# CliMA/ClimaSeaIce.jl

Hardware: AMD Instinct MI355X
Metric: EVP sub-cycle cell-updates/s (higher is better)
Workload: dtype f64; 1 GPU; evp_subcycle_fplane_periodic_2048x2048_as_1x1_tiles_of_2048x2048_120substeps; substeps=120, mode=fast, halo=4, halo_exchange=none (one tile)

## Files before the change

climaseaice.jl_amd/csrc/evp_fast_math.h:

```cpp
#pragma once
#include "csi_dev.h"

namespace csi {
namespace fm {

#define CSI_EPS64 2.220446049250313e-16

__device__ __forceinline__ double fma_(double a, double b, double c) { return __builtin_fma(a, b, c); }
__device__ __forceinline__ double fmax_(double a, double b) { return __builtin_fmax(a, b); }
__device__ __forceinline__ double fmin_(double a, double b) { return __builtin_fmin(a, b); }
__device__ __forceinline__ double clampd(double x, double lo, double hi) { return x > hi ? hi : (x < lo ? lo : x); }
__device__ __forceinline__ double avg2(double a, double b) { return 0.5 * (a + b); }
__device__ __forceinline__ double avg4(double a, double b, double c, double d) { return 0.25 * ((a + b) + (c + d)); }
__device__ __forceinline__ double sum2(double a, double b) { return a + b; }
__device__ __forceinline__ double quarter(double s_a, double s_b) { return 0.25 * (s_a + s_b); }

__device__ __forceinline__ double rcp(double x) {
    const double r = __builtin_amdgcn_rcp(x);
    return fma_(fma_(-x, r, 1.0), r, r);
}
__device__ __forceinline__ double rsqrt(double x) {
    const double y = __builtin_amdgcn_rsq(x);
    const double g = x * y, h = 0.5 * y;
    const double r = fma_(-h, g, 0.5);
    return fma_(y, r, y);
}
__device__ __forceinline__ void sqrt_rsqrt(double x, double& s, double& rs) {
    const double y = __builtin_amdgcn_rsq(x);
    double g = x * y, h = 0.5 * y;
    const double r = fma_(-h, g, 0.5);
    g = fma_(g, r, g);
    h = fma_(h, r, h);
    const double d = fma_(-g, g, x);
    s = fma_(d, h, g);
    rs = 2.0 * h;
}
__device__ __forceinline__ double sqrt_fast(double x) {
    const double y = __builtin_amdgcn_rsq(x);
    const double g = x * y, h = 0.5 * y;
    const double r = fma_(-h, g, 0.5);
    return fma_(g, r, g);
}

template <bool UNI>
__device__ __forceinline__ void strain_cell(double A, double Bn, double Bs, double Cn, double Cs,
                                            double u_e, double u_w, double v_n, double v_s, double& e11, double& e22) {
    if (UNI) {
        e11 = A * (u_e - u_w);
        e22 = Cn * (v_n - v_s);
    } else {
        e11 = fma_(A, u_e - u_w, fma_(Bn, v_n, -(Bs * v_s)));
        e22 = fma_(Cn, v_n, -(Cs * v_s));
    }
}
template <bool UNI>
__device__ __forceinline__ double strain_corner(double Sn, double Ss, double Sv, double u_n, double u_s, double v_e, double v_w) {
    if (UNI) return fma_(Sv, v_e - v_w, Sn * (u_n - u_s));
    return fma_(Sv, v_e - v_w, fma_(Sn, u_n, -(Ss * u_s)));
}

struct StressConst {
    double em2, Dmin, Dmin2, rDmin, amin, amax, amin2, amax2, ramin, ramax;
    double hk1;
    int pressure_kind;
    double em2_8, Dmin2_16;
};

struct StressOut {
    double s11, s22, s12, alpha, zc2, zf2;
    double xc, rDc;
};

__device__ __forceinline__ StressOut stress_update_r(const StressConst& k, double e11c, double e22c, double e12f,
                                                     double e11f, double e22f, double e12c, double Pc, double Pf,
                                                     double mc, double mf, double rmc, double rmf, double hkc, double hkf,
                                                     double s11, double s22, double s12) {
    StressOut o;
    const double dc = e11c + e22c, df = e11f + e22f;
    const double tc = e11c - e22c, tf = e11f - e22f;
    const double sc2 = fma_(tc, tc, 4.0 * (e12c * e12c));
    const double sf2 = fma_(tf, tf, 4.0 * (e12f * e12f));
    const double xc = fmax_(fma_(dc, dc, sc2 * k.em2), k.Dmin2), xf = fmax_(fma_(df, df, sf2 * k.em2), k.Dmin2);
    const double rDc = rsqrt(xc), rDf = rsqrt(xf);
    const double zc2 = Pc * rDc, zf2 = Pf * rDf;
    const double Pr = (k.pressure_kind == 0) ? Pc * rcp(fma_(k.Dmin, rDc, 1.0)) : Pc;
    const double ec2 = zc2 * k.em2, ef2 = zf2 * k.em2;
    const double bulk = fma_(zc2 * k.hk1, dc, -0.5 * Pr);
    const double s11n = fma_(ec2, e11c, bulk);
    const double s22n = fma_(ec2, e22c, bulk);
    const double s12n = ef2 * e12f;
    const double g2c_raw = zc2 * hkc * rmc, g2f_raw = zf2 * hkf * rmf;
    const double g2c = fmax_(fmin_(g2c_raw, k.amax2), k.amin2);
    const double g2f = fmax_(fmin_(g2f_raw, k.amax2), k.amin2);
    double gc, rgc, gf, rgf;
    sqrt_rsqrt(g2c, gc, rgc);
    sqrt_rsqrt(g2f, gf, rgf);
    const double wc = (mc > 0) ? rgc : 0.0, wf = (mf > 0) ? rgf : 0.0;
    o.s11 = fma_(s11n - s11, wc, s11);
    o.s22 = fma_(s22n - s22, wc, s22);
    o.s12 = fma_(s12n - s12, wf, s12);
    o.alpha = gc;
    o.zc2 = zc2; o.zf2 = zf2; o.xc = xc; o.rDc = rDc;
    return o;
}

__device__ __forceinline__ StressOut stress_update_s(const StressConst& k, double e11c, double e22c, double E12f,
                                                     double S11f, double S22f, double y2, double Pc, double XP,
                                                     double mc, double M4, double rmc, double rM4, double hkc, double hkf4,
                                                     double s11, double s22, double s12) {
    StressOut o;
    const double dc = e11c + e22c, DF = S11f + S22f;
    const double tc = e11c - e22c, TF = S11f - S22f;
    const double sc2 = fma_(tc, tc, y2 * y2);
    const double sf2 = fma_(TF, TF, E12f * E12f);
    const double xc = fmax_(fma_(dc, dc, sc2 * k.em2), k.Dmin2), xf = fmax_(fma_(DF, DF, sf2 * k.em2), k.Dmin2_16);
    const double rDc = rsqrt(xc), rDf = rsqrt(xf);
    const double zc2 = Pc * rDc, zf2 = XP * rDf;
    const double Pr = (k.pressure_kind == 0) ? Pc * rcp(fma_(k.Dmin, rDc, 1.0)) : Pc;
    const double ec2 = zc2 * k.em2, ef2 = zf2 * k.em2_8;
    const double bulk = fma_(zc2 * k.hk1, dc, -0.5 * Pr);
    const double s11n = fma_(ec2, e11c, bulk);
    const double s22n = fma_(ec2, e22c, bulk);
    const double s12n = ef2 * E12f;
    const double g2c_raw = zc2 * hkc * rmc, g2f_raw = zf2 * hkf4 * rM4;
    const double g2c = fmax_(fmin_(g2c_raw, k.amax2), k.amin2);
    const double g2f = fmax_(fmin_(g2f_raw, k.amax2), k.amin2);
    double gc, rgc, gf, rgf;
    sqrt_rsqrt(g2c, gc, rgc);
    sqrt_rsqrt(g2f, gf, rgf);
    const double wc = (mc > 0) ? rgc : 0.0, wf = (M4 > 0) ? rgf : 0.0;
    o.s11 = fma_(s11n - s11, wc, s11);
    o.s22 = fma_(s22n - s22, wc, s22);
    o.s12 = fma_(s12n - s12, wf, s12);
    o.alpha = gc;
    o.zc2 = zc2; o.zf2 = zf2; o.xc = xc; o.rDc = rDc;
    return o;
}

__device__ __forceinline__ StressOut stress_update(const StressConst& k, double e11c, double e22c, double e12f,
                                                   double e11f, double e22f, double e12c, double Pc, double Pf,
                                                   double mc, double mf, double hkc, double hkf,
                                                   double s11, double s22, double s12) {
    return stress_update_r(k, e11c, e22c, e12f, e11f, e22f, e12c, Pc, Pf, mc, mf, rcp(mc), rcp(mf), hkc, hkf, s11, s22, s12);
}

struct VelConst {
    double dt, rdt, fcor, min_mass, min_conc;
    int has_cor;
};

__device__ __forceinline__ void ext_stress(int kind, double tau, double rhoCd, double we, double webar, double w, double wbar,
                                           double& ex, double& im) {
    if (kind == 3) {
        const double d1 = we - w, d2 = webar - wbar;
        const double n2 = fma_(d1, d1, d2 * d2);
        const double n = sqrt_fast(fmax_(n2, 2.2250738585072014e-308));
        im = rhoCd * n;
        ex = im * we;
    } else {
        ex = tau; im = 0.0;
    }
}

__device__ __forceinline__ void ext_stress_rest(double rhoCd, double w, double wbar, double& ex, double& im) {
    const double n2 = fma_(w, w, wbar * wbar);
    im = rhoCd * sqrt_fast(fmax_(n2, 2.2250738585072014e-308));
    ex = 0.0;
}

__device__ __forceinline__ double vel_update_avg(const VelConst& k, double w, double wn, double mi, double ai, double abar,
                                                 double div, double cor, double ext, double imt, double exb, double imb, bool peripheral) {
    const double rm = rcp(mi);
    const double rai = rm * ai;
    const double G = fma_(wn - w, k.rdt, fma_(div, rm, fma_(exb - ext, rai, cor)));
    const double tau_i = (imb - imt) * rai;
    const double wD = fma_(k.dt, G, abar * w) * rcp(fma_(k.dt, tau_i, abar));
    const bool active_ice = (mi >= k.min_mass) & (ai >= k.min_conc);
    double res = active_ice ? wD : 0.0;
    return peripheral ? 0.0 : res;
}
__device__ __forceinline__ double vel_update_avg_fd(const VelConst& k, double w, double wn, double mi, double ai, double abar,
                                                    double div, double cor, double ext, double imt, double exb, double imb,
                                                    bool peripheral, double wf) {
    const double wD = vel_update_avg(k, w, wn, mi, ai, abar, div, cor, ext, imt, exb, imb, false);
    const bool active_ice = (mi >= k.min_mass) & (ai >= k.min_conc);
    const bool marginal = (mi > CSI_EPS64) & (ai > CSI_EPS64);
    const double res = active_ice ? wD : (marginal ? wf : 0.0);
    return peripheral ? 0.0 : res;
}
__device__ __forceinline__ double vel_update(const VelConst& k, double w, double wn, double m_a, double m_b, double a_a, double a_b,
                                             double al_a, double al_b, double div, double cor,
                                             double ext, double imt, double exb, double imb, bool peripheral) {
    return vel_update_avg(k, w, wn, avg2(m_a, m_b), avg2(a_a, a_b), avg2(al_a, al_b), div, cor, ext, imt, exb, imb, peripheral);
}
__device__ __forceinline__ double vel_update_fd(const VelConst& k, double w, double wn, double m_a, double m_b, double a_a, double a_b,
                                                double al_a, double al_b, double div, double cor,
                                                double ext, double imt, double exb, double imb, bool peripheral, double wf) {
    return vel_update_avg_fd(k, w, wn, avg2(m_a, m_b), avg2(a_a, a_b), avg2(al_a, al_b), div, cor, ext, imt, exb, imb, peripheral, wf);
}

__device__ __forceinline__ double vel_update_sum(const VelConst& k2, double w, double wn, double m2, double a2, double al2,
                                                 double div2, double cor, double ext, double imt, double exb, double imb, bool peripheral) {
    const double rm2 = rcp(m2);
    const double rai = rm2 * a2;
    const double G = fma_(wn - w, k2.rdt, fma_(div2, rm2, fma_(exb - ext, rai, cor)));
    const double tau_i = (imb - imt) * rai;
    const double wD = fma_(k2.dt, G, al2 * w) * rcp(fma_(k2.dt, tau_i, al2));
    const bool active_ice = (m2 >= k2.min_mass) & (a2 >= k2.min_conc);
    double res = active_ice ? wD : 0.0;
    return peripheral ? 0.0 : res;
}
__device__ __forceinline__ double vel_update_sum_fd(const VelConst& k2, double w, double wn, double m2, double a2, double al2,
                                                    double div2, double cor, double ext, double imt, double exb, double imb,
                                                    bool peripheral, double wf) {
    const double wD = vel_update_sum(k2, w, wn, m2, a2, al2, div2, cor, ext, imt, exb, imb, false);
    const bool active_ice = (m2 >= k2.min_mass) & (a2 >= k2.min_conc);
    const bool marginal = (m2 > 2.0 * CSI_EPS64) & (a2 > 2.0 * CSI_EPS64);
    const double res = active_ice ? wD : (marginal ? wf : 0.0);
    return peripheral ? 0.0 : res;
}

__device__ __forceinline__ double div1(double E, double Fn, double Fs, double s11_0, double s11_m, double s12_p, double s12_0) {
    return fma_(E, s11_0 - s11_m, fma_(Fn, s12_p, -(Fs * s12_0)));
}
template <bool UNI>
__device__ __forceinline__ double div2(double Q1n, double Q2n, double Q1s, double Q2s, double K,
                                       double s11_0, double s22_0, double s11_m, double s22_m, double s12_p, double s12_0) {
    if (UNI) return fma_(K, s12_p - s12_0, Q2n * (s22_0 - s22_m));
    const double n = fma_(Q1n, s11_0, Q2n * s22_0);
    const double s = fma_(Q1s, s11_m, Q2s * s22_m);
    return fma_(K, s12_p - s12_0, n - s);
}

__device__ __forceinline__ void full_strain_cell(double Uy_e, double Uy_w, double Vx_n, double Vx_s, double Ur_e, double Ur_w,
                                                 double Vr_n, double Vr_s, double dyc2, double dxc2, double razc, double& e11, double& e22) {
    const double D1 = (Uy_e - Uy_w) + (Vx_n - Vx_s);
    const double D2 = fma_(dyc2, Ur_e - Ur_w, -(dxc2 * (Vr_n - Vr_s)));
    const double hr = 0.5 * razc;
    e11 = hr * (D1 + D2);
    e22 = hr * (D1 - D2);
}
__device__ __forceinline__ double full_strain_corner(double Ux_n, double Ux_s, double Vy_e, double Vy_w, double dxf2, double dyf2, double razf) {
    return (0.5 * razf) * fma_(dxf2, Ux_n - Ux_s, dyf2 * (Vy_e - Vy_w));
}
__device__ __forceinline__ double full_div1(double dyu, double rdyu, double rdxu, double razu, double S_e, double S_w, double T_e, double T_w,
                                            double Z_n, double Z_s) {
    return razu * fma_(0.5 * dyu, S_e - S_w, fma_(0.5 * rdyu, T_e - T_w, rdxu * (Z_n - Z_s)));
}
__device__ __forceinline__ double full_div2(double dxv, double rdxv, double rdyv, double razv, double S_n, double S_s, double T_n, double T_s,
                                            double Z_e, double Z_w) {
    return razv * fma_(0.5 * dxv, S_n - S_s, fma_(-0.5 * rdxv, T_n - T_s, rdyv * (Z_e - Z_w)));
}

__device__ __forceinline__ double full_strain_corner8(double Ux_n, double Ux_s, double Vy_e, double Vy_w, double dxf2, double dyf2, double razf) {
    return (4.0 * razf) * fma_(dxf2, Ux_n - Ux_s, dyf2 * (Vy_e - Vy_w));
}
__device__ __forceinline__ double full_div1_x2(double dyu, double rdyu, double rdxu, double razu, double S_e, double S_w, double T_e, double T_w,
                                               double Z_n, double Z_s) {
    return razu * fma_(dyu, S_e - S_w, fma_(rdyu, T_e - T_w, (rdxu + rdxu) * (Z_n - Z_s)));
}
__device__ __forceinline__ double full_div2_x2(double dxv, double rdxv, double rdyv, double razv, double S_n, double S_s, double T_n, double T_s,
                                               double Z_e, double Z_w) {
    return razv * fma_(dxv, S_n - S_s, fma_(-rdxv, T_n - T_s, (rdyv + rdyv) * (Z_e - Z_w)));
}

}
}
```

climaseaice.jl_amd/csrc/evp_fused2.hip:

```cpp
#include "evp_pair_stage.h"

#include <cstdio>
#include <cstdlib>

#ifndef CSI_PAIR_WAVES
#define CSI_PAIR_WAVES 3
#endif
#ifndef CSI_PAIR_UNI_WAVES
#define CSI_PAIR_UNI_WAVES 2
#endif
#ifndef CSI_PAIR_FULL_WAVES
#define CSI_PAIR_FULL_WAVES 2
#endif
#ifndef CSI_PAIR_PRIO
#define CSI_PAIR_PRIO 2
#endif
#ifndef CSI_PAIR_HOIST
#define CSI_PAIR_HOIST 1
#endif
#ifndef CSI_FULL_FENCE
#define CSI_FULL_FENCE 1
#endif
#ifndef CSI_PAIR_STORES
#define CSI_PAIR_STORES 7
#endif
#ifndef CSI_PEER_EXP
#define CSI_PEER_EXP 3
#endif
#ifndef CSI_PAIR_SKIPB
#define CSI_PAIR_SKIPB 0
#endif
#ifndef CSI_PAIR_PD
#define CSI_PAIR_PD 1
#endif

namespace csi {
namespace fused {

#ifdef CSI_PAIR_PROBE
static __device__ unsigned long long g_probe[8192 * 16];
#define PROBE_DECL unsigned long long pacc0 = 0, pacc1 = 0, pacc2 = 0, ptprev = 0, pit = 0; const unsigned long long pwall0 = wall_clock64()
#define PROBE_START do { __builtin_amdgcn_sched_barrier(0); ptprev = __builtin_readcyclecounter(); __builtin_amdgcn_sched_barrier(0); ++pit; } while (0)
#define PROBE(acc) do { __builtin_amdgcn_sched_barrier(0); const unsigned long long t_ = __builtin_readcyclecounter(); \
                        __builtin_amdgcn_sched_barrier(0); acc += t_ - ptprev; ptprev = t_; } while (0)
#define PROBE_END(slot) do { if (lane == 0 && (slot) < 8192 && !write_diag) { unsigned long long* dbg = g_probe + (size_t)(slot) * 16; \
                        dbg[0] = pacc0; dbg[1] = pacc1; dbg[2] = pacc2; dbg[6] = pit; dbg[8] = pwall0; dbg[9] = wall_clock64(); \
                        dbg[12] = PSTAGE.sp0; dbg[13] = PSTAGE.sp1; dbg[14] = PSTAGE.sp2; dbg[15] = PSTAGE.sp3; \
                        dbg[10] = (unsigned long long)__builtin_amdgcn_s_getreg((31 << 11) | (0 << 6) | 4); dbg[11] = (unsigned long long)blockIdx.x; } } while (0)
#else
#define PROBE_DECL do { } while (0)
#define PROBE_START do { } while (0)
#define PROBE(acc) do { } while (0)
#define PROBE_END(slot) do { } while (0)
#endif

template <int V> struct Idx { static constexpr int value = V; };

constexpr int RING_ROWS = 4;
enum : int { RF_S11 = 0, RF_S22, RF_S12, RF_U, RF_V, RF_P, RF_M, RF_A, RF_UN, RF_VN, RF_PF, RF_RMC, RF_RMF };
#ifndef CSI_PAIR_LDSC_NOPRE
#define CSI_PAIR_LDSC_NOPRE 1
#endif
#ifndef CSI_PAIR_PRE
#define CSI_PAIR_PRE 1
#endif
#ifndef CSI_PAIR_FRING
#define CSI_PAIR_FRING 1
#endif
constexpr int RF_FORCING = 8;
enum : int { RF_FU_TAU = 10, RF_FU_WE, RF_FU_WB, RF_FU_FD, RF_FV_TAU, RF_FV_WE, RF_FV_WB, RF_FV_FD };
constexpr int RP_ROWS = 3, RP_FIELDS = 12;
enum : int { RP_DXV = 0, RP_RDYV, RP_RDXU, RP_DXF2, RP_DYF2, RP_RAZF, RP_DYU, RP_DYC2, RP_DXC2, RP_RAZC, RP_RAZU, RP_RAZV };

template <bool UNI, bool AUF, bool WALLS, bool MASK, bool FORCE, bool FD, int CF, bool FULL = false, bool PEER = false, int EXTRA = 0, bool DLD = false>
__device__ __forceinline__ void pair_body(const FusedTable* __restrict__ table, const int w, int nstrips, int nchunks, int rows,
                                       int blocks_per_xcd, int write_diag, unsigned long long seq,
                                       double* __restrict__ ring, unsigned* __restrict__ ringm, double* __restrict__ outr, unsigned* __restrict__ peer_abort_p, double* __restrict__ ringp,
                                       double* __restrict__ ringc) {
    constexpr bool LDSC = !UNI && !FULL && !(EXTRA == 1 && MASK) && (CSI_PAIR_LDSC != 0);
    constexpr bool FRING = FORCE && !FULL && (EXTRA != 1 || !MASK) && CSI_PAIR_FRING;
    constexpr bool PRE = CSI_PAIR_PRE && !MASK && !FULL && !FRING && !(CSI_PAIR_LDSC_NOPRE && !UNI && !(EXTRA == 1 && MASK) && (CSI_PAIR_LDSC != 0));
    constexpr int RING_FIELDS = FRING ? 10 + RF_FORCING : (PRE ? 13 : 10);
#define peer_abort (*peer_abort_p)
    const int b = (int)blockIdx.x;
#ifndef CSI_EXP_ROLESWAP
#define CSI_EXP_ROLESWAP 0
#endif
    const bool consumer = (__builtin_amdgcn_readfirstlane((int)(threadIdx.x >> 6)) != 0) != (CSI_EXP_ROLESWAP && ((((b >> 3) / CSI_EXP_ROLESWAP) & 1) != 0));
    const int chunk = w / nstrips, strip = w - chunk * nstrips;
    const int lane = (int)(threadIdx.x & 63);
    tptr_t T = (tptr_t)table;
    const bool single = (write_diag & 2) != 0;
    write_diag &= 1;

    int ja, jb, rstart, rend;
    unsigned loff, sc, sf;
    unsigned lm = 0, sm = 0;
    int i;
    unsigned flags;
    int dx;
    int dxv;
    bool wave_valx_b = false;
    bool wave_has_dx_b;
    bool lanes_uniform;
    bool lanes_same;
    int row0;
    enum : unsigned { L_RS = 1, L_R1 = 2, L_R2 = 4, L_WALL_U = 8, L_WALL_V = 16, L_MIR_LO = 32, L_MIR_HI = 64, L_VAL_LO = 128, L_VAL_HI = 256, L_LOW = 512 };
    {
        const int Nx = T->I[FI_NX], Hx = T->I[FI_HX], Hy = T->I[FI_HY];
        const int i0s = T->I[FI_DEC + 0] - P_LO + strip * P_W;
        i = i0s + lane;
        {
            const int elo = T->I[FI_ELO] > 0 ? T->I[FI_ELO] : rows;
            ja = (T->I[FI_EHI] > 0 && chunk == nchunks - 1 && chunk > 0) ? T->I[FI_DEC + 3] - T->I[FI_EHI] + 1
                                                                         : T->I[FI_DEC + 2] + (chunk == 0 ? 0 : elo + (chunk - 1) * rows);
            jb = chunk == 0 ? min(ja + elo - 1, T->I[FI_DEC + 3])
                            : (chunk == nchunks - 1 ? T->I[FI_DEC + 3] : min(ja + rows - 1, T->I[FI_DEC + 3] - T->I[FI_EHI]));
        }
        const int ic = min(max(i, 1 - Hx), Nx + Hx);
        loff = (unsigned)(ic - (1 - Hx)) * 8u;
        row0 = 1 - Hy;
        const bool own = (lane >= P_LO) & (lane <= P_HI) & (i <= T->I[FI_DEC + 1]);
        flags = 0;
        if (own & (i >= T->I[FI_RS + 0]) & (i <= T->I[FI_RS + 1])) flags |= L_RS;
        if (own & (i >= T->I[FI_R1 + 0]) & (i <= T->I[FI_R1 + 1])) flags |= L_R1;
        if (own & (i >= T->I[FI_R2 + 0]) & (i <= T->I[FI_R2 + 1])) flags |= L_R2;
        dx = 0;
        if ((T->I[FI_XLO] == SIDE_PERIODIC) & (i >= 1) & (i <= Hx)) dx = Nx * 8;
        else if ((T->I[FI_XHI] == SIDE_PERIODIC) & (i > Nx - Hx) & (i <= Nx)) dx = -Nx * 8;
        dxv = dx;
        if (WALLS) {
            const bool xlo_wall = T->I[FI_XLO] == SIDE_WALL, xhi_wall = T->I[FI_XHI] == SIDE_WALL;
            if ((xlo_wall & (i <= 1)) | (xhi_wall & (i > Nx))) flags |= L_WALL_U;
            if ((xlo_wall & (i < 1)) | (xhi_wall & (i > Nx))) flags |= L_WALL_V;
            if (xlo_wall & (i == 0)) flags |= L_MIR_LO;
            if (xhi_wall & (i == Nx + 1)) flags |= L_MIR_HI;
            const bool vval_lo = T->I[FI_IMV + 0] == IMG_VALUE, vval_hi = T->I[FI_IMV + 1] == IMG_VALUE;
            if (xlo_wall & (i >= 1) & (i <= Hx)) dxv = vval_lo ? ((i == 1) ? -8 : 0) : (1 - 2 * i) * 8;
            if (xhi_wall & (i > Nx - Hx) & (i <= Nx)) dxv = vval_hi ? ((i == Nx) ? 8 : 0) : (2 * Nx + 1 - 2 * i) * 8;
            if (xlo_wall & vval_lo & ((i == 1) | (i == 0))) flags |= L_VAL_LO;
            if (xhi_wall & vval_hi & ((i == Nx) | (i == Nx + 1))) flags |= L_VAL_HI;
            wave_valx_b = __builtin_amdgcn_ballot_w64((flags & (L_VAL_LO | L_VAL_HI)) != 0) != 0;
        }
        wave_has_dx_b = __builtin_amdgcn_ballot_w64((dx != 0) | (dxv != 0)) != 0;
        const bool same = ((flags & L_RS) != 0) == ((flags & L_R1) != 0) && ((flags & L_RS) != 0) == ((flags & L_R2) != 0);
        lanes_same = __builtin_amdgcn_ballot_w64(!same) == 0;
        lanes_uniform = !wave_has_dx_b && lanes_same;
        rstart = max(ja - 3, T->I[FI_AJ0]);
#ifndef CSI_EXP_RINGCUT
#define CSI_EXP_RINGCUT 0
#endif
        rend = min(jb + 3 - CSI_EXP_RINGCUT, T->I[FI_AJ1]);
        if (i <= Hx) flags |= L_LOW;
        sc = (unsigned)T->I[FI_LD_C] * 8u;
        sf = (unsigned)T->I[FI_LD_F] * 8u;
        if (MASK) {
            sm = (unsigned)T->I[FI_MASK_LD];
            lm = (unsigned)(ic - (1 - Hx));
        }
    }
    unsigned pdirs = 0;
    if constexpr (PEER) {
        const bool pw = strip < T->I[FI_PSET], pe = strip >= nstrips - T->I[FI_PSET + 1], ps = chunk < T->I[FI_PSET + 2],
                   pn = chunk >= nchunks - T->I[FI_PSET + 3];
        pdirs = ((pw ? 1u : 0u) | (pe ? 2u : 0u) | (ps ? 4u : 0u) | (pn ? 8u : 0u) | ((ps & pw) ? 16u : 0u) | ((ps & pe) ? 32u : 0u) |
                 ((pn & pw) ? 64u : 0u) | ((pn & pe) ? 128u : 0u)) & (unsigned)T->I[FI_PMASK];
        pdirs = (unsigned)__builtin_amdgcn_readfirstlane((int)pdirs);
        if (pdirs) {
            if (!consumer && !(CSI_PEER_EXP & 4)) {
                const unsigned long long t0 = wall_clock64();
                bool dead = false;
                for (;;) {
                    bool behind = false, poison = false;
                    if constexpr ((CSI_PEER_EXP & 8) != 0) {
                        const unsigned long long* slots = (const unsigned long long*)T->P[FP_SLOT_IN + 2];
                        if (lane < 15) {
                            const int cq = (chunk + lane / 3 - 2 + 2 * nchunks) % nchunks, cs = (strip + lane % 3 - 1 + nstrips) % nstrips;
                            behind |= __hip_atomic_load(slots + (cq * nstrips + cs), __ATOMIC_RELAXED, __HIP_MEMORY_SCOPE_SYSTEM) + 1ull < seq;
                        }
                    } else
#pragma unroll
                    for (int d = 0; d < 8; ++d) {
                        if (!((pdirs >> d) & 1u)) continue;
                        const int nslots = T->I[FI_PWAIT + d];
                        const unsigned long long* slots = (const unsigned long long*)T->P[FP_SLOT_IN + d];
#pragma unroll 1
                        for (int b0 = 0; b0 < nslots; b0 += 64) {
                            const int idx = b0 + lane;
                            if (idx < nslots) behind |= __hip_atomic_load(slots + idx, __ATOMIC_RELAXED, __HIP_MEMORY_SCOPE_SYSTEM) + 1ull < seq;
                        }
                        if (lane == 63) poison |= __hip_atomic_load(slots + (kPeerSlots - 1), __ATOMIC_RELAXED, __HIP_MEMORY_SCOPE_SYSTEM) != 0ull;
                    }
                    if (__builtin_amdgcn_ballot_w64(behind) == 0) break;
                    if (__builtin_amdgcn_ballot_w64(poison | (*(volatile unsigned*)T->P[FP_PERR] != 0u)) != 0 || wall_clock64() - t0 > 300000000ull) { dead = true; break; }
                    __builtin_amdgcn_s_sleep(8);
                }
                if (dead) {
                    if (lane == 0) *(volatile unsigned*)T->P[FP_PERR] = 1u;
                    if (lane < 8) {
                        typedef const __attribute__((address_space(4))) unsigned long* sptr_t;
                        unsigned long long* out = (unsigned long long*)((sptr_t)&T->P[FP_SLOT_OUT])[lane];
                        if (out) __hip_atomic_store(out + (kPeerSlots - 1), 1ull, __ATOMIC_RELAXED, __HIP_MEMORY_SCOPE_SYSTEM);
                    }
                }
                if (lane == 0) peer_abort = dead ? 1u : 0u;
                if (T->I[FI_PTIER] >= 1) __builtin_amdgcn_fence(__ATOMIC_ACQUIRE, "");
                __builtin_amdgcn_sched_barrier(0);
            }
            __syncthreads();
            if (peer_abort) return;
        }
    }
    auto offc = [&](int j) __attribute__((always_inline)) { return loff + (unsigned)(j - row0) * sc; };
    auto offf = [&](int j) __attribute__((always_inline)) { return loff + (unsigned)(j - row0) * sf; };
    auto offm = [&](int j) __attribute__((always_inline)) { return lm + (unsigned)(j - row0) * sm; };
    const int NyW = T->I[FI_NY], HyW = T->I[FI_HY];
    int rcd = 0;
    if constexpr (FULL) {
        typedef const __attribute__((address_space(4))) int* iptr_t;
        iptr_t rcs = (iptr_t)T->P[FP_RCSUM];
        if (rcs) {
            const int t0 = max(rstart - 4, row0) - row0, t1 = min(rend + 2, NyW + HyW + 1) - row0;
            if (rcs[t1 + 1] - rcs[t0] == t1 - t0 + 1) rcd = FP_C2ROW_0 - FP_C2_0;
        }
    }
    const unsigned c2s = FULL ? (rcd ? 8u : (unsigned)T->I[FI_C2_LD] * 8u) : 0u;
    const unsigned loff2 = (FULL && rcd) ? 0u : loff;
    auto off2 = [&](int j) __attribute__((always_inline)) { return loff2 + (unsigned)(j - row0) * c2s; };
    const int NyLoW = PEER ? T->I[FI_NYLO] : NyW;
    const bool wrap_lo_b = T->I[FI_YLO] == SIDE_PERIODIC, wrap_hi_b = T->I[FI_YHI] == SIDE_PERIODIC;
    const bool ylo_wall_b = WALLS && T->I[FI_YLO] == SIDE_WALL, yhi_wall_b = WALLS && T->I[FI_YHI] == SIDE_WALL;
    const bool uval_lo_b = WALLS && T->I[FI_IMU + 2] == IMG_VALUE, uval_hi_b = WALLS && T->I[FI_IMU + 3] == IMG_VALUE;
    enum : unsigned { U_WRAPLO = 1, U_YLO = 2, U_YHI = 4, U_UVLO = 8, U_UVHI = 16, U_HASDX = 32, U_VALX = 64, U_WRAPHI = 128, U_MIR = 256 };
    const bool wave_mir_b = WALLS && __builtin_amdgcn_ballot_w64((flags & (L_MIR_LO | L_MIR_HI)) != 0) != 0;
    const unsigned UF = (unsigned)__builtin_amdgcn_readfirstlane((int)((wrap_lo_b ? U_WRAPLO : 0u) | (wrap_hi_b ? U_WRAPHI : 0u) | (ylo_wall_b ? U_YLO : 0u) | (yhi_wall_b ? U_YHI : 0u) |
                                                                         (uval_lo_b ? U_UVLO : 0u) | (uval_hi_b ? U_UVHI : 0u) |
                                                                         (wave_has_dx_b ? U_HASDX : 0u) | (wave_valx_b ? U_VALX : 0u) | (wave_mir_b ? U_MIR : 0u)));
#define wrap_lo ((UF & U_WRAPLO) != 0)
#define wrap_hi ((UF & U_WRAPHI) != 0)
#define ylo_wall (WALLS && (UF & U_YLO) != 0)
#define yhi_wall (WALLS && (UF & U_YHI) != 0)
#define uval_lo (WALLS && (UF & U_UVLO) != 0)
#define uval_hi (WALLS && (UF & U_UVHI) != 0)
#define wave_has_dx ((UF & U_HASDX) != 0)
#define wave_valx (WALLS && (UF & U_VALX) != 0)
#define wave_mir (WALLS && (UF & U_MIR) != 0)
#define has_dld (PEER && DLD)
    auto wall_row = [&](int j) __attribute__((always_inline)) { return (ylo_wall & (j < 1)) | (yhi_wall & (j > NyW)); };
    auto wall_vrow = [&](int j) __attribute__((always_inline)) { return (ylo_wall & (j <= 1)) | (yhi_wall & (j > NyW)); };
    const bool lane_wu = WALLS && (flags & L_WALL_U) != 0, lane_wv = WALLS && (flags & L_WALL_V) != 0;
    auto numbers = [&](Forcing& F) __attribute__((always_inline)) {
        F.t_tau_u = T->K[FK_TOP_TAU_U]; F.t_we_u = T->K[FK_TOP_UE]; F.t_wb_u = T->K[FK_TOP_VE];
        F.b_tau_u = T->K[FK_BOT_TAU_U]; F.b_we_u = T->K[FK_BOT_UE]; F.b_wb_u = T->K[FK_BOT_VE];
        F.t_tau_v = T->K[FK_TOP_TAU_V]; F.t_we_v = T->K[FK_TOP_VE]; F.t_wb_v = T->K[FK_TOP_UE];
        F.b_tau_v = T->K[FK_BOT_TAU_V]; F.b_we_v = T->K[FK_BOT_VE]; F.b_wb_v = T->K[FK_BOT_UE];
        F.fd_u = 0.0; F.fd_v = 0.0; F.fd = FD;
        F.xc_u = 0.0; F.xd_u = 0.0; F.xc_v = 0.0; F.xd_v = 0.0; F.extra = EXTRA == 1 ? T->I[FI_EXTRA] : 0;
    };
    auto arrays = [&](Forcing& F, unsigned ou, unsigned ov) __attribute__((always_inline)) {
        if (T->I[FI_TOP_KIND] == 2) { F.t_tau_u = ldg(T->P[FP_FT_U], ou); F.t_tau_v = ldg(T->P[FP_FT_V], ov); }
        if constexpr (EXTRA == 2) {
            if (T->I[FI_TOP_UEK] == 2) { F.t_we_u = ldg(T->P[FP_FT_U], ou); F.t_wb_v = ldg(T->P[FP_FT_UBAR], ov); }
            if (T->I[FI_TOP_VEK] == 2) { F.t_we_v = ldg(T->P[FP_FT_V], ov); F.t_wb_u = ldg(T->P[FP_FT_VBAR], ou); }
            if (T->I[FI_BOT_KIND] == 2) { F.b_tau_u = ldg(T->P[FP_FB_U], ou); F.b_tau_v = ldg(T->P[FP_FB_V], ov); }
        }
        if (T->I[FI_BOT_UEK] == 2) { F.b_we_u = ldg(T->P[FP_FB_U], ou); F.b_wb_v = ldg(T->P[FP_FB_UBAR], ov); }
        if (T->I[FI_BOT_VEK] == 2) { F.b_we_v = ldg(T->P[FP_FB_V], ov); F.b_wb_u = ldg(T->P[FP_FB_VBAR], ou); }
        if (FD) { F.fd_u = ldg(T->P[FP_FD_U], ou); F.fd_v = ldg(T->P[FP_FD_V], ov); }
        if (EXTRA == 1) {
            if (F.extra & 1) { F.xc_u = ldg(T->P[FP_XC_U], ou); F.xc_v = ldg(T->P[FP_XC_V], ov); }
            if (F.extra & 2) { F.xd_u = ldg(T->P[FP_XD_U], ou); F.xd_v = ldg(T->P[FP_XD_V], ov); }
        }
    };
    auto stress_consts = [&](fm::StressConst& ks) __attribute__((always_inline)) {
        ks.em2 = T->K[FK_EM2]; ks.Dmin = T->K[FK_DMIN]; ks.Dmin2 = T->K[FK_DMIN2]; ks.rDmin = T->K[FK_RDMIN];
        ks.amin = T->K[FK_AMIN]; ks.amax = T->K[FK_AMAX]; ks.amin2 = T->K[FK_AMIN2]; ks.amax2 = T->K[FK_AMAX2];
        ks.ramin = T->K[FK_RAMIN]; ks.ramax = T->K[FK_RAMAX]; ks.hk1 = T->K[FK_HK1]; ks.pressure_kind = T->I[FI_PRESSURE_KIND];
        ks.em2_8 = T->K[FK_PK_EM2_8]; ks.Dmin2_16 = T->K[FK_PK_DMIN2_16];
    };
    auto vel_consts = [&](fm::VelConst& kv) __attribute__((always_inline)) {
        kv.dt = T->K[FK_DT2]; kv.rdt = T->K[FK_RDT]; kv.fcor = T->K[FK_FCOR]; kv.min_mass = T->K[FK_MIN_MASS2];
        kv.min_conc = T->K[FK_MIN_CONC2]; kv.has_cor = T->I[FI_HAS_COR];
    };
    const int prio_rank = (int)(__builtin_amdgcn_s_getreg((3 << 11) | (0 << 6) | 4) % 3u);
    auto set_prio = [&](int k) __attribute__((always_inline)) {
        if (CSI_PAIR_PRIO == 2) {
            if (consumer) __builtin_amdgcn_s_setprio(2); else __builtin_amdgcn_s_setprio(0);
        } else if (CSI_PAIR_PRIO == 3) {
            if (consumer) __builtin_amdgcn_s_setprio(0); else __builtin_amdgcn_s_setprio(2);
        } else if (CSI_PAIR_PRIO == 4) {
            if (consumer) __builtin_amdgcn_s_setprio(3); else __builtin_amdgcn_s_setprio(0);
        } else if (CSI_PAIR_PRIO) {
            int p = prio_rank + k;
            p = p >= 3 ? p - 3 : p;
            if (p == 0) __builtin_amdgcn_s_setprio(0); else if (p == 1) __builtin_amdgcn_s_setprio(1); else __builtin_amdgcn_s_setprio(2);
        }
    };
    const int rs_lo = max(ja, T->I[FI_RS + 2]), rs_hi = min(jb, T->I[FI_RS + 3]);
    const int r1_lo = max(ja, T->I[FI_R1 + 2]), r1_hi = min(jb, T->I[FI_R1 + 3]);
    const int r2_lo = max(ja, T->I[FI_R2 + 2]), r2_hi = min(jb, T->I[FI_R2 + 3]);
    auto yimg = [&](int j) __attribute__((always_inline)) {
        return (wrap_lo & (j >= 1) & (j <= HyW)) ? NyLoW : ((wrap_hi & (j > NyW - HyW) & (j <= NyW)) ? -NyW : 0);
    };
    auto yimg_u = [&](int j) __attribute__((always_inline)) {
        int d = yimg(j);
        if (WALLS) {
            if (ylo_wall & (j >= 1) & (j <= HyW)) d = uval_lo ? ((j == 1) ? -1 : 0) : 1 - 2 * j;
            if (yhi_wall & (j > NyW - HyW) & (j <= NyW)) d = uval_hi ? ((j == NyW) ? 1 : 0) : 2 * NyW + 1 - 2 * j;
        }
        return d;
    };
    enum : int { D_W = 0, D_E, D_S, D_N, D_SW, D_SE, D_NW, D_NE };
    auto own = [&](int k) __attribute__((always_inline)) { return T->P[k < 5 ? FP_S11_OUT + k : FP_AL + (k - 5)]; };
    auto img = [&](int k, int d) __attribute__((always_inline)) { return PEER ? T->P[FP_IMG0 + d * 9 + k] : own(k); };
    const bool wave_low = PEER && __builtin_amdgcn_ballot_w64(((flags & L_LOW) != 0) & ((dx != 0) | (dxv != 0))) != 0;
    const bool wt = T->I[FI_WT] != 0;
    auto sto = [&](unsigned long b_, unsigned o_, double v_) __attribute__((always_inline)) {
        if (wt) stg_agent(b_, o_, v_); else stg(b_, o_, v_);
    };
    auto put4 = [&](int k, unsigned off, unsigned dy, bool ylow, int dxl, double val, double valy, double valx, double valxy, int j, int yr) __attribute__((always_inline)) {
        const unsigned long base = own(k);
        auto sti = [&](unsigned long b_, unsigned o_, double v_) __attribute__((always_inline)) {
            if constexpr (PEER && (CSI_PEER_EXP & 2) != 0)
                __scoped_atomic_store_n((__attribute__((address_space(1))) long*)((gptr_t)b_ + o_), __builtin_bit_cast(long, v_), __ATOMIC_RELAXED, __MEMORY_SCOPE_SYSTEM);
            else sto(b_, o_, v_);
        };
        sto(base, off, val);
        if constexpr (PEER) {
            if (has_dld) {
                const int cls = (k == 2 || k == 3 || k == 7) ? 1 : 0;
                const int p0 = j + HyW - 1, p1 = p0 + yr;
                const int dY = ylow ? D_S : D_N, dX = wave_low ? D_W : D_E;
                const int dXY = ylow ? (wave_low ? D_SW : D_SE) : (wave_low ? D_NW : D_NE);
                if (dy != 0u) sti(img(k, dY), off + dy + (unsigned)(p1 * T->I[FI_PDLD + dY * 2 + cls]), valy);
                if (wave_has_dx && dxl != 0) {
                    sti(img(k, dX), off + (unsigned)dxl + (unsigned)(p0 * T->I[FI_PDLD + dX * 2 + cls]), valx);
                    if (dy != 0u) sti(img(k, dXY), off + (unsigned)dxl + dy + (unsigned)(p1 * T->I[FI_PDLD + dXY * 2 + cls]), valxy);
                }
                return;
            }
        }
        if (dy != 0u) sti(PEER ? (ylow ? img(k, D_S) : img(k, D_N)) : base, off + dy, valy);
        if (wave_has_dx) {
            if (dxl != 0) {
                sti(PEER ? (wave_low ? img(k, D_W) : img(k, D_E)) : base, off + (unsigned)dxl, valx);
                if (dy != 0u) sti(PEER ? (ylow ? (wave_low ? img(k, D_SW) : img(k, D_SE)) : (wave_low ? img(k, D_NW) : img(k, D_NE))) : base, off + (unsigned)dxl + dy, valxy);
            }
        }
    };
    auto put = [&](int k, unsigned off, unsigned dy, bool ylow, int dxl, double val, int j, int yr) __attribute__((always_inline)) {
        put4(k, off, dy, ylow, dxl, val, val, val, val, j, yr);
    };
    auto put_u = [&](unsigned off, int j, unsigned dy, double val, int yr) __attribute__((always_inline)) {
        double vy = val;
        if (WALLS) {
            if (uval_lo & ylo_wall & (j == 1)) vy = 2 * T->K[FK_BCU] - val;
            if (uval_hi & yhi_wall & (j == NyW)) vy = 2 * T->K[FK_BCU + 1] - val;
        }
        put4(3, off, dy, j <= HyW, dx, val, vy, val, vy, j, yr);
    };
    auto put_v = [&](unsigned off, unsigned dy, bool ylow, double val, int j, int yr) __attribute__((always_inline)) {
        double vx = val;
        if (WALLS && wave_valx) {
            if (flags & L_VAL_LO) vx = 2 * T->K[FK_BCV] - val;
            if (flags & L_VAL_HI) vx = 2 * T->K[FK_BCV + 1] - val;
        }
        put4(4, off, dy, ylow, dxv, val, val, vx, vx, j, yr);
    };
    int fast_lo, fast_hi;
    {
        const int d1 = AUF ? 0 : 1;
        fast_lo = max(rs_lo, max(r1_lo + d1, r2_lo + 1));
        fast_hi = min(rs_hi, min(r1_hi + d1, r2_hi + 1));
        if (wrap_lo | ylo_wall) fast_lo = max(fast_lo, HyW + 2);
        if (wrap_hi | yhi_wall) fast_hi = min(fast_hi, NyW - HyW);
    }
    const bool fast_plain = lanes_uniform;
    auto flush = [&](int q, double v11, double v22, double v12, double vfirst, double vsecond, auto WH, auto VFT) __attribute__((always_inline)) {
        constexpr int which = decltype(WH)::value;
        constexpr bool VF = decltype(VFT)::value != 0;
        if (which == 0) return;
        if ((q >= fast_lo) & (q <= fast_hi)) {
            const unsigned ocq = offc(q), ofq = offf(q);
            if (fast_plain) {
                if (flags & L_RS) {
                    if (which & 1) { sto(T->P[FP_S11_OUT], ocq, v11); sto(T->P[FP_S22_OUT], ocq, v22); sto(T->P[FP_S12_OUT], ofq, v12); }
                    if (which & 2) sto(T->P[VF ? FP_V_OUTP : FP_U_OUTP], VF ? ocq : ofq - sf, vfirst);
                    if (which & 4) sto(T->P[VF ? FP_U_OUTP : FP_V_OUTP], VF ? ofq - sf : ocq - sc, vsecond);
                }
            } else {
                const bool ls = (flags & L_RS) != 0, l1 = (flags & L_R1) != 0, l2 = (flags & L_R2) != 0;
                if ((which & 1) && ls) { put(0, ocq, 0u, false, dx, v11, q, 0); put(1, ocq, 0u, false, dx, v22, q, 0); put(2, ofq, 0u, false, dx, v12, q, 0); }
                if (VF) { if ((which & 2) && l1) put_v(ocq, 0u, false, vfirst, q, 0); if ((which & 4) && l2) put(3, ofq - sf, 0u, false, dx, vsecond, q - 1, 0); }
                else { if ((which & 2) && l1) put(3, ofq - sf, 0u, false, dx, vfirst, q - 1, 0); if ((which & 4) && l2) put_v(ocq - sc, 0u, false, vsecond, q - 1, 0); }
            }
            return;
        }
        const int j1 = VF ? q : q - 1, j2 = q - 1;
        const bool do_s = ((which & 1) != 0) & (q >= rs_lo) & (q <= rs_hi), do_1 = ((which & 2) != 0) & (j1 >= r1_lo) & (j1 <= r1_hi),
                   do_2 = ((which & 4) != 0) & (j2 >= r2_lo) & (j2 <= r2_hi);
        if (!(do_s | do_1 | do_2)) return;
        const unsigned ocq = offc(q), ofq = offf(q);
        const unsigned o1 = VF ? ocq : ofq - sf;
        const unsigned o2 = VF ? ofq - sf : ocq - sc;
        const int yq = yimg(q), y1 = VF ? yimg(j1) : yimg_u(j1), y2 = VF ? yimg_u(j2) : yimg(j2);
        if (do_s & ((flags & L_RS) != 0)) {
            put(0, ocq, (unsigned)yq * sc, q <= HyW, dx, v11, q, yq);
            put(1, ocq, (unsigned)yq * sc, q <= HyW, dx, v22, q, yq);
            put(2, ofq, (unsigned)yq * sf, q <= HyW, dx, v12, q, yq);
        }
        if (do_1 & ((flags & L_R1) != 0)) {
            if (VF) put_v(o1, (unsigned)y1 * sc, j1 <= HyW, vfirst, j1, y1); else put_u(o1, j1, (unsigned)y1 * sf, vfirst, y1);
        }
        if (do_2 & ((flags & L_R2) != 0)) {
            if (VF) put_u(o2, j2, (unsigned)y2 * sf, vsecond, y2); else put_v(o2, (unsigned)y2 * sc, j2 <= HyW, vsecond, j2, y2);
        }
    };
    unsigned lane_it = (unsigned)lane;
    auto fresh_lane = [&]() __attribute__((always_inline)) {
        if constexpr (MASK && !FULL) {
            unsigned l;
            asm volatile("v_mbcnt_lo_u32_b32 %0, -1, 0\n\tv_mbcnt_hi_u32_b32 %0, -1, %0" : "=v"(l));
            lane_it = l;
        }
    };
    auto rslot = [&](int j) __attribute__((always_inline)) { return (unsigned)((j - rstart) & (RING_ROWS - 1)) * (RING_FIELDS * 64) + lane_it; };

#ifndef CSI_PAIR_UNROLL
#define CSI_PAIR_UNROLL 3
#endif

    if (!consumer) {
        PROBE_DECL;
        Stage<UNI, AUF, MASK, FORCE, CF, FULL, !(EXTRA == 1 && MASK)> A;
        A.lc = ringc;
        const int cjmin = LDSC ? T->I[FI_COEF_JMIN] : 0, cjmax = LDSC ? T->I[FI_COEF_JMAX] : 0;
        const unsigned ck_lane = (unsigned)min(lane, FC_COUNT - 1) * 8u;
        auto coef_row_base = [&](int j) __attribute__((always_inline)) {
            return T->P[FP_PCOEF_VEC] + (unsigned long)((long)min(max(j, cjmin), cjmax) * (long)(FC_COUNT * 8));
        };
#ifndef CSI_EXP_RINGALIAS
#define CSI_EXP_RINGALIAS 0
#endif
        auto alias_row = [&](int j) __attribute__((always_inline)) { return CSI_EXP_RINGALIAS ? min(max(j, ja + 1), max(jb - 1, ja + 1)) : j; };
        unsigned oc = offc(alias_row(rstart)), of = offf(alias_row(rstart)), om = MASK ? offm(rstart) : 0u;
        {
            const double rho0 = T->K[FK_RHO];
            A.u_m = ldg(T->P[FP_U_IN], of - sf); A.v_m = ldg(T->P[FP_V_IN], oc - sc);
            A.u_0 = ldg(T->P[FP_U_IN], of); A.v_0 = ldg(T->P[FP_V_IN], oc);
            A.a_mm = 0.0; A.a_m = ldg(T->P[FP_A], oc - sc);
            A.m_mm = 0.0; A.m_m = ldg(T->P[FP_H], oc - sc) * rho0 * A.a_m;
            const double P_m = ldg(T->P[FP_P], oc - sc);
            A.XP_m = fm::sum2(from_left(P_m), P_m);
            A.Xm_m = fm::sum2(from_left(A.m_m), A.m_m);
            A.Xa_m = fm::sum2(from_left(A.a_m), A.a_m);
            A.Xv_m = fm::sum2(from_left(A.v_m), A.v_m);
            A.Xv_0 = fm::sum2(from_left(A.v_0), A.v_0);
            double e11_m, e22_m;
            const int jm = rstart - 1;
            A.hoist_uniform(T);
            if constexpr (FULL) {
                const unsigned om2 = off2(jm), o02 = off2(rstart);
                full_cell(T, om2, c2s, A.u_m, A.v_m, A.v_0, e11_m, e22_m, rcd);
                A.e12_0 = 8.0 * full_corner(T, o02, c2s, A.u_0, A.u_m, A.v_0, rcd);
                A.hoist_planes(T, rcd);
                A.full_init(T, o02, om2, c2s);
            } else {
            fm::strain_cell<UNI>(pcoef<UNI>(T, FC_A, jm), pcoef<UNI>(T, FC_BN, jm), pcoef<UNI>(T, FC_BS, jm), pcoef<UNI>(T, FC_CN, jm),
                            pcoef<UNI>(T, FC_CS, jm), from_right(A.u_m), A.u_m, A.v_0, A.v_m, e11_m, e22_m);
            A.e12_0 = fm::strain_corner<UNI>(pcoef<UNI>(T, FC_SN, rstart), pcoef<UNI>(T, FC_SS, rstart), pcoef<UNI>(T, FC_SV, rstart), A.u_0, A.u_m, A.v_0, from_left(A.v_0));
            }
            A.Xe11_m = fm::sum2(from_left(e11_m), e11_m);
            A.Xe22_m = fm::sum2(from_left(e22_m), e22_m);
            A.Ye12_0 = fm::sum2(A.e12_0, from_right(A.e12_0));
            A.XAL_m = 0; A.XS11L_m = 0; A.XS22L_m = 0; A.XW = 0; A.Wprev = 0;
            A.S11_mm = 0; A.S22_mm = 0; A.S12_mm = 0; A.AL_mm = 0; A.S11_m = 0; A.S22_m = 0; A.S12_m = 0; A.AL_m = 0;
            A.S11_0 = 0; A.S22_0 = 0; A.S12_0 = 0; A.AL_0 = 0; A.first = 0; A.second = 0;
        }
#pragma unroll
        for (int q = 0; q < RING_ROWS * RING_FIELDS; ++q) ring[q * 64 + lane] = 0.0;
        if constexpr (FULL) {
#pragma unroll
            for (int q = 0; q < RP_ROWS * RP_FIELDS; ++q) ringp[q * 64 + lane] = 1.0;
            A.RAZU_m = 1.0; A.RAZV_x = 1.0; A.RAZC_0 = 1.0;
        }
        unsigned mhist = 0xffffffffu;
        if (MASK) {
            const bool wi = lane_wv | wall_row(rstart - 1);
            const unsigned act = ldub(T->P[FP_MASK], om - sm);
            mhist = (mhist << 2) | (wi ? 3u : (act ? 0u : 1u));
            ringm[(unsigned)((-1) & (RING_ROWS - 1)) * 64 + (unsigned)lane] = mhist & 3u;
        }
        RowIn R[3];
#ifndef CSI_FULL_HOISTP
#define CSI_FULL_HOISTP 1
#endif
#ifndef CSI_FORCE_HOIST
#define CSI_FORCE_HOIST 0
#endif
        constexpr bool HIN = (FULL && CSI_FULL_HOISTP >= 2) || (FORCE && !FULL && (CSI_FORCE_HOIST & 1));
        const unsigned long hU = HIN ? T->P[FP_U_IN] : 0ul, hV = HIN ? T->P[FP_V_IN] : 0ul, hP = HIN ? T->P[FP_P] : 0ul, hH = HIN ? T->P[FP_H] : 0ul,
                            hA = HIN ? T->P[FP_A] : 0ul, h11 = HIN ? T->P[FP_S11_IN] : 0ul, h22 = HIN ? T->P[FP_S22_IN] : 0ul, h12 = HIN ? T->P[FP_S12_IN] : 0ul,
                            hUN = HIN ? T->P[FP_UN] : 0ul, hVN = HIN ? T->P[FP_VN] : 0ul;
        int rnext = rstart;
        auto load_row = [&](RowIn& Q) __attribute__((always_inline)) {
            if constexpr (HIN) {
                Q.u_p = ldg(hU, of + sf); Q.v_p = ldg(hV, oc + sc);
                Q.P_0 = ldg(hP, oc); Q.h_0 = ldg(hH, oc); Q.a_0 = ldg(hA, oc);
                Q.s11 = ldg(h11, oc); Q.s22 = ldg(h22, oc); Q.s12 = ldg(h12, of);
                Q.un_m = ldg(hUN, of - sf); Q.vn_x = ldg(hVN, AUF ? oc - sc : oc);
            } else {
            Q.u_p = ldg(T->P[FP_U_IN], of + sf); Q.v_p = ldg(T->P[FP_V_IN], oc + sc);
            Q.P_0 = ldg(T->P[FP_P], oc); Q.h_0 = ldg(T->P[FP_H], oc); Q.a_0 = ldg(T->P[FP_A], oc);
            Q.s11 = ldg(T->P[FP_S11_IN], oc); Q.s22 = ldg(T->P[FP_S22_IN], oc); Q.s12 = ldg(T->P[FP_S12_IN], of);
            Q.un_m = ldg(T->P[FP_UN], of - sf); Q.vn_x = ldg(T->P[FP_VN], AUF ? oc - sc : oc);
            }
            Q.mk = MASK ? ldub(T->P[FP_MASK], om) : 1u;
            if constexpr (LDSC) Q.ck = ldg(coef_row_base(rnext + 2), ck_lane);
        };
        auto advance = [&]() __attribute__((always_inline)) {
            const bool more = rnext < rend;
            if (CSI_EXP_RINGALIAS) { rnext += more ? 1 : 0; oc = offc(alias_row(rnext)); of = offf(alias_row(rnext)); return; }
            oc += more ? sc : 0u; of += more ? sf : 0u;
            if (MASK) om += more ? sm : 0u;
            rnext += more ? 1 : 0;
        };
        int r = rstart;
        auto body = [&](auto KK) __attribute__((always_inline)) {
            constexpr int k = decltype(KK)::value;
            if (!CSI_PAIR_HOIST || FORCE || (FULL && CSI_FULL_FENCE)) asm volatile("" : "+s"(T));
            set_prio(k);
            fresh_lane();
            PROBE_START;
            if (CSI_PAIR_PD == 1) __builtin_amdgcn_s_waitcnt(0x0F70);
            else if (MASK) __builtin_amdgcn_s_waitcnt(0x0F70 | 11);
            else __builtin_amdgcn_s_waitcnt(0x0F70 | 10);
            PROBE(pacc0);
            const RowIn& C = R[k];
            if constexpr (LDSC) { if (lane < FC_COUNT) ringc[(unsigned)((r + 2) & 7) * FC_COUNT + (unsigned)lane] = C.ck; }
            const unsigned so = (unsigned)((r - rstart) & 1) * (5 * 64) + (unsigned)lane;
            constexpr int PW = 7 & ~CSI_PAIR_STORES;
            double o11 = 0, o22 = 0, o12 = 0, ofirst = 0, osecond = 0;
            if (PW & 1) { o11 = outr[so]; o22 = outr[so + 64]; o12 = outr[so + 128]; }
            if (PW & 2) ofirst = outr[so + 192];
            if (PW & 4) osecond = outr[so + 256];
            Forcing FA;
            numbers(FA);
            if (FORCE) arrays(FA, offf(r - 1), AUF ? offc(r - 1) : offc(r));
            if constexpr (!FULL) {
                advance();
                load_row(R[(k + CSI_PAIR_PD) % 3]);
            }
            flush(r - 4, o11, o22, o12, ofirst, osecond, Idx<PW>{}, Idx<AUF ? 1 : 0>{});
            fm::StressConst ks; stress_consts(ks);
            fm::VelConst kv; vel_consts(kv);
            const double m_0 = C.h_0 * T->K[FK_RHO] * C.a_0;
            const bool pa1 = WALLS && (AUF ? (lane_wu | wall_row(r - 1)) : (lane_wv | wall_vrow(r)));
            const bool pa2 = WALLS && (AUF ? (lane_wv | wall_vrow(r - 1)) : (lane_wu | wall_row(r - 1)));
            if (MASK) {
                const bool wi = lane_wv | wall_row(r);
                mhist = (mhist << 2) | (wi ? 3u : (C.mk ? 0u : 1u));
            }
            if constexpr (FULL) {
                static_assert(CSI_PAIR_PD == 1, "the per-point-metric producer prefetches one row ahead");
                auto mid = [&]() __attribute__((always_inline)) { advance(); load_row(R[(k + 1) % 3]); };
                A.template step<false>(T, ks, kv, r, C.u_p, C.v_p, C.P_0, m_0, C.a_0, C.s11, C.s22, C.s12, C.un_m, C.vn_x, true, r > rstart, pa1, pa2, mhist, FA,
                                       off2(r), c2s, off2(min(r + 1, rend)), off2(max(r - 1, row0)), mid);
            } else
            A.step(T, ks, kv, r, C.u_p, C.v_p, C.P_0, m_0, C.a_0, C.s11, C.s22, C.s12, C.un_m, C.vn_x, true, r > rstart, pa1, pa2, mhist, FA);
            {
                const unsigned s0 = rslot(r), s1 = rslot(r - 1);
                ring[s0 + RF_S11 * 64] = A.S11_0; ring[s0 + RF_S22 * 64] = A.S22_0; ring[s0 + RF_S12 * 64] = A.S12_0;
                if (AUF) { ring[s1 + RF_U * 64] = A.first; ring[s1 + RF_V * 64] = A.second; }
                else { ring[s0 + RF_V * 64] = A.first; ring[s1 + RF_U * 64] = A.second; }
                if (single) {
                    ring[s0 + RF_P * 64] = A.AL_0; ring[s0 + RF_M * 64] = 0.5 * A.zf; ring[s0 + RF_A * 64] = 0.5 * A.zc; ring[s0 + RF_VN * 64] = A.Dc * A.rDc;
                } else {
                ring[s0 + RF_P * 64] = C.P_0; ring[s0 + RF_M * 64] = m_0; ring[s0 + RF_A * 64] = C.a_0;
                if (PRE) { ring[s0 + RF_PF * 64] = A.Pf_0; ring[s0 + RF_RMC * 64] = A.rmc_0; ring[s0 + RF_RMF * 64] = A.rmf_0; }
                ring[s1 + RF_UN * 64] = C.un_m; ring[(AUF ? s1 : s0) + RF_VN * 64] = C.vn_x;
                }
                if constexpr (FRING) {
                    if constexpr (EXTRA == 2) {
                        const bool tt = T->I[FI_TOP_KIND] == 2, bt = T->I[FI_BOT_KIND] == 2;
                        ring[s0 + RF_FU_TAU * 64] = tt ? FA.t_tau_u : FA.t_we_u; ring[s0 + RF_FU_FD * 64] = FA.t_wb_u;
                        ring[s0 + RF_FU_WE * 64] = bt ? FA.b_tau_u : FA.b_we_u; ring[s0 + RF_FU_WB * 64] = FA.b_wb_u;
                        ring[s0 + RF_FV_TAU * 64] = tt ? FA.t_tau_v : FA.t_we_v; ring[s0 + RF_FV_FD * 64] = FA.t_wb_v;
                        ring[s0 + RF_FV_WE * 64] = bt ? FA.b_tau_v : FA.b_we_v; ring[s0 + RF_FV_WB * 64] = FA.b_wb_v;
                    } else {
                    ring[s0 + RF_FU_TAU * 64] = FA.t_tau_u; ring[s0 + RF_FU_WE * 64] = FA.b_we_u; ring[s0 + RF_FU_WB * 64] = FA.b_wb_u; ring[s0 + RF_FU_FD * 64] = EXTRA == 1 ? FA.xc_u : FA.fd_u;
                    ring[s0 + RF_FV_TAU * 64] = FA.t_tau_v; ring[s0 + RF_FV_WE * 64] = FA.b_we_v; ring[s0 + RF_FV_WB * 64] = FA.b_wb_v; ring[s0 + RF_FV_FD * 64] = EXTRA == 1 ? FA.xc_v : FA.fd_v;
                    }
                }
                if constexpr (FULL) {
                    const unsigned p0 = (unsigned)k * (RP_FIELDS * 64) + lane_it;
                    ringp[p0 + RP_DXV * 64] = A.DXV_p; ringp[p0 + RP_RDYV * 64] = A.RDYV_p; ringp[p0 + RP_RDXU * 64] = A.RDXU_p;
                    ringp[p0 + RP_DXF2 * 64] = A.DXF2_p; ringp[p0 + RP_DYF2 * 64] = A.DYF2_p; ringp[p0 + RP_RAZF * 64] = A.RAZF_p;
                    ringp[p0 + RP_DYU * 64] = A.DYU_0; ringp[p0 + RP_DYC2 * 64] = A.DYC2_0; ringp[p0 + RP_DXC2 * 64] = A.DXC2_0;
                    ringp[p0 + RP_RAZC * 64] = A.RAZC_0; ringp[p0 + RP_RAZU * 64] = A.RAZU_m; ringp[p0 + RP_RAZV * 64] = A.RAZV_x;
                }
                if (MASK) ringm[(unsigned)((r - rstart) & (RING_ROWS - 1)) * 64 + lane_it] = mhist & 3u;
            }
            A.shift(C.u_p, C.v_p, m_0, C.a_0);
            PROBE(pacc1);
#ifndef CSI_EXP_HALFBARRIER
#define CSI_EXP_HALFBARRIER 0
#endif
            if (!(CSI_EXP_HALFBARRIER && ((r - rstart) & 1)))
            __syncthreads();
            PROBE(pacc2);
        };
        if constexpr (LDSC) {
#pragma unroll
            for (int d = -3; d <= 1; ++d) {
                const double v = ldg(coef_row_base(rstart + d), ck_lane);
                if (lane < FC_COUNT) ringc[(unsigned)((rstart + d) & 7) * FC_COUNT + (unsigned)lane] = v;
            }
        }
        load_row(R[0]);
        if (CSI_PAIR_PD == 2) {
            advance();
            load_row(R[1]);
        }
        for (;;) {
            body(Idx<0>{});
            if (++r > rend) break;
            body(Idx<1>{});
            if (++r > rend) break;
            body(Idx<2>{});
            if (++r > rend) break;
        }
        for (int d = 0; d < 2; ++d) {
            const unsigned so = (unsigned)((r - rstart) & 1) * (5 * 64) + (unsigned)lane;
            flush(r - 4, outr[so], outr[so + 64], outr[so + 128], outr[so + 192], outr[so + 256], Idx<(7 & ~CSI_PAIR_STORES)>{}, Idx<AUF ? 1 : 0>{});
            if (d == 0) __syncthreads();
            ++r;
        }
#define PSTAGE A
        PROBE_END(w * 2);
#undef PSTAGE
        return;
    }

    auto publish = [&]() __attribute__((always_inline)) {
        if (PEER && pdirs) {
            if ((CSI_PEER_EXP & 1) && T->I[FI_PTIER] < 2) __builtin_amdgcn_s_waitcnt(0x0F70);
            else { __builtin_amdgcn_fence(__ATOMIC_RELEASE, ""); asm volatile("s_waitcnt vmcnt(0)" ::: "memory"); }
            if ((lane < 8) && ((pdirs >> lane) & 1u)) {
                const int nW = T->I[FI_PSET], nE = T->I[FI_PSET + 1], nN = T->I[FI_PSET + 3];
                const bool xw = (lane == D_W) | (lane == D_SW) | (lane == D_NW), xe = (lane == D_E) | (lane == D_SE) | (lane == D_NE);
                const bool yn = (lane == D_N) | (lane == D_NW) | (lane == D_NE);
                const int xs = xe ? strip - (nstrips - nE) : strip, xn = xw ? nW : (xe ? nE : nstrips);
                const int ys = yn ? chunk - (nchunks - nN) : chunk;
                typedef const __attribute__((address_space(4))) unsigned long* sptr_t;
                unsigned long long* out = (unsigned long long*)((sptr_t)&T->P[FP_SLOT_OUT])[lane];
                __hip_atomic_store(out + (ys * xn + xs), seq, __ATOMIC_RELAXED, __HIP_MEMORY_SCOPE_SYSTEM);
            }
        }
    };

    if (single) {
        {
            const int d1 = AUF ? 1 : 0;
            fast_lo = max(rs_lo, max(r1_lo + d1, r2_lo + 1));
            fast_hi = min(rs_hi, min(r1_hi + d1, r2_hi + 1));
            if (wrap_lo | ylo_wall) fast_lo = max(fast_lo, HyW + 2);
            if (wrap_hi | yhi_wall) fast_hi = min(fast_hi, NyW - HyW);
            }
        for (int r = rstart; r <= rend; ++r) {
            __syncthreads();
            const unsigned s0 = rslot(r), s1 = rslot(r - 1);
            const double v11 = ring[s0 + RF_S11 * 64], v22 = ring[s0 + RF_S22 * 64], v12 = ring[s0 + RF_S12 * 64];
            const double vfirst = AUF ? ring[s1 + RF_U * 64] : ring[s0 + RF_V * 64];
            const double vsecond = AUF ? ring[s1 + RF_V * 64] : ring[s1 + RF_U * 64];
            const double dal = ring[s0 + RF_P * 64], dzf = ring[s0 + RF_M * 64], dzc = ring[s0 + RF_A * 64], ddl = ring[s0 + RF_VN * 64];
            flush(r, v11, v22, v12, vfirst, vsecond, Idx<7>{}, Idx<AUF ? 0 : 1>{});
            if (write_diag) {
                if (((flags & L_RS) != 0) & (r >= rs_lo) & (r <= rs_hi)) {
                    const unsigned ocq = offc(r), ofq = offf(r);
                    const int yq = yimg(r);
                    put(5, ocq, (unsigned)yq * sc, r <= HyW, dx, dal, r, yq);
                    put(7, ofq, (unsigned)yq * sf, r <= HyW, dx, dzf, r, yq);
                    put(6, ocq, (unsigned)yq * sc, r <= HyW, dx, dzc, r, yq);
                    put(8, ocq, (unsigned)yq * sc, r <= HyW, dx, ddl, r, yq);
                }
            }
        }
        __syncthreads();
        publish();
        return;
    }

    PROBE_DECL;
    Stage<UNI, !AUF, MASK, FORCE, CF, FULL, !(EXTRA == 1 && MASK)> B;
    B.lc = ringc;
    B.u_m = 0; B.u_0 = 0; B.v_m = 0; B.v_0 = 0; B.Xv_m = 0; B.Xv_0 = 0;
    B.a_mm = 0; B.a_m = 0; B.m_mm = 0; B.m_m = 0;
    B.XP_m = 0; B.Xm_m = 0; B.Xa_m = 0; B.Xe11_m = 0; B.Xe22_m = 0; B.Ye12_0 = 0; B.e12_0 = 0;
    B.XAL_m = 0; B.XS11L_m = 0; B.XS22L_m = 0; B.XW = 0; B.Wprev = 0;
    B.S11_mm = 0; B.S22_mm = 0; B.S12_mm = 0; B.AL_mm = 0; B.S11_m = 0; B.S22_m = 0; B.S12_m = 0; B.AL_m = 0;
    B.S11_0 = 0; B.S22_0 = 0; B.S12_0 = 0; B.AL_0 = 0; B.first = 0; B.second = 0;
    B.zc = 0; B.zf = 0; B.Dc = 0; B.rDc = 0; B.Pf_0 = 0; B.rmc_0 = 0; B.rmf_0 = 0;
    B.hoist_uniform(T);
    if constexpr (FULL) {
        B.hoist_planes(T, rcd);
        B.full_init(T, off2(max(rstart - 2, row0)), off2(max(rstart - 3, row0)), c2s);
        B.full_prefetch_vel(T, off2(max(rstart - 2, row0)), off2(max(rstart - 3, row0)));
    }
    int fq = 0;
    bool fhave = false;
    double f11 = 0, f22 = 0, f12 = 0, ffirst = 0, fsecond = 0;
    const int rlo = rstart - 1;
    unsigned mhistB = 0xffffffffu;
    double vn_delay = 0.0;
    double razv_delay = 1.0;
    double fvd_tau = 0.0, fvd_we = 0.0, fvd_wb = 0.0, fvd_fd = 0.0;
    int r = rstart;
    auto bodyB = [&](auto KK) __attribute__((always_inline)) {
        if (!CSI_PAIR_HOIST || FORCE || (FULL && CSI_FULL_FENCE)) asm volatile("" : "+s"(T));
        set_prio(decltype(KK)::value);
        const int q = r - 2;
        PROBE_START;
        if (!(CSI_EXP_HALFBARRIER && ((r - rstart) & 1)))
        __syncthreads();
        PROBE(pacc0);
        if constexpr (!FULL && CSI_PAIR_SKIPB) { if (q < ja - 3) return; }
        fresh_lane();
        const unsigned s1 = rslot(r - 1), s2 = rslot(r - 2), s3 = rslot(r - 3);
        double bu_p = ring[s1 + RF_U * 64], bv_p = ring[s1 + RF_V * 64];
        const double s11 = ring[s2 + RF_S11 * 64], s22 = ring[s2 + RF_S22 * 64], s12 = ring[s2 + RF_S12 * 64];
        const double bP_0 = ring[s2 + RF_P * 64], bm_0 = ring[s2 + RF_M * 64], ba_0 = ring[s2 + RF_A * 64];
        if (PRE) { B.Pf_0 = ring[s2 + RF_PF * 64]; B.rmc_0 = ring[s2 + RF_RMC * 64]; B.rmf_0 = ring[s2 + RF_RMF * 64]; }
        const double bun = ring[s3 + RF_UN * 64], vn_new = ring[s2 + RF_VN * 64];
        const double bvn = AUF ? vn_new : vn_delay;
        vn_delay = vn_new;
        const unsigned bmk = MASK ? ringm[(unsigned)((r - 2 - rstart) & (RING_ROWS - 1)) * 64 + lane_it] : 0u;
        if constexpr (FULL) {
            if (fhave) flush(fq, f11, f22, f12, ffirst, fsecond, Idx<(CSI_PAIR_STORES & 7)>{}, Idx<AUF ? 1 : 0>{});
        }
        PROBE(pacc1);
        fm::StressConst ks; stress_consts(ks);
        fm::VelConst kv; vel_consts(kv);
        if (WALLS) {
            if (wave_mir) {
            const double vl = from_left(bv_p), vr = from_right(bv_p);
            double ml = vr, mh = vl;
            if (wave_valx) {
                if (flags & L_VAL_LO) ml = 2 * T->K[FK_BCV] - vr;
                if (flags & L_VAL_HI) mh = 2 * T->K[FK_BCV + 1] - vl;
            }
            bv_p = (flags & L_MIR_LO) ? ml : ((flags & L_MIR_HI) ? mh : bv_p);
            }
            if (ylo_wall & (q == 0)) B.u_0 = uval_lo ? 2 * T->K[FK_BCU] - bu_p : bu_p;
            if (yhi_wall & (q == NyW)) bu_p = uval_hi ? 2 * T->K[FK_BCU + 1] - B.u_0 : B.u_0;
        }
        if (MASK) mhistB = (mhistB << 2) | ((q >= rlo) ? bmk : 3u);
        Forcing FB;
        numbers(FB);
        if constexpr (FRING) {
            const double u0 = ring[s2 + RF_FU_TAU * 64], u1 = ring[s2 + RF_FU_WE * 64], u2 = ring[s2 + RF_FU_WB * 64], u3 = ring[s2 + RF_FU_FD * 64];
            double v0, v1, v2, v3;
            if (AUF) {
                v0 = ring[s1 + RF_FV_TAU * 64]; v1 = ring[s1 + RF_FV_WE * 64]; v2 = ring[s1 + RF_FV_WB * 64]; v3 = ring[s1 + RF_FV_FD * 64];
            } else {
                const double n0 = ring[s2 + RF_FV_TAU * 64], n1 = ring[s2 + RF_FV_WE * 64], n2 = ring[s2 + RF_FV_WB * 64], n3 = ring[s2 + RF_FV_FD * 64];
                v0 = fvd_tau; v1 = fvd_we; v2 = fvd_wb; v3 = fvd_fd;
                fvd_tau = n0; fvd_we = n1; fvd_wb = n2; fvd_fd = n3;
            }
            if constexpr (EXTRA == 2) {
                if (T->I[FI_TOP_KIND] == 2) { FB.t_tau_u = u0; FB.t_tau_v = v0; } else { FB.t_we_u = u0; FB.t_we_v = v0; }
                FB.t_wb_u = u3; FB.t_wb_v = v3;
                if (T->I[FI_BOT_KIND] == 2) { FB.b_tau_u = u1; FB.b_tau_v = v1; } else { FB.b_we_u = u1; FB.b_we_v = v1; }
                FB.b_wb_u = u2; FB.b_wb_v = v2;
            } else {
                FB.t_tau_u = u0; FB.b_we_u = u1; FB.b_wb_u = u2;
                FB.t_tau_v = v0; FB.b_we_v = v1; FB.b_wb_v = v2;
                if (EXTRA == 1) { FB.xc_u = u3; FB.xc_v = v3; } else { FB.fd_u = u3; FB.fd_v = v3; }
            }
        } else if (FORCE) {
            const int qm = max(q - 1, row0), qa = max(q, row0);
#ifndef CSI_EXP_NOCONSLOADS
            arrays(FB, offf(qm), AUF ? offc(qa) : offc(qm));
#endif
        }
        const bool pb1 = WALLS && (!AUF ? (lane_wu | wall_row(q - 1)) : (lane_wv | wall_vrow(q)));
        const bool pb2 = WALLS && (!AUF ? (lane_wv | wall_vrow(q - 1)) : (lane_wu | wall_row(q - 1)));
        if constexpr (FULL) {
            constexpr int kk = decltype(KK)::value;
            auto midB = [&]() __attribute__((always_inline)) {
                const unsigned pn = (unsigned)((kk + 2) % 3) * (RP_FIELDS * 64) + lane_it;
                B.N_DXV = ringp[pn + RP_DXV * 64]; B.N_RDYV = ringp[pn + RP_RDYV * 64]; B.N_RDXU = ringp[pn + RP_RDXU * 64];
                B.N_DXF2 = ringp[pn + RP_DXF2 * 64]; B.N_DYF2 = ringp[pn + RP_DYF2 * 64]; B.N_RAZF = ringp[pn + RP_RAZF * 64];
                B.N_DYU = ringp[pn + RP_DYU * 64]; B.N_DYC2 = ringp[pn + RP_DYC2 * 64]; B.N_DXC2 = ringp[pn + RP_DXC2 * 64];
                B.N_RAZC = ringp[pn + RP_RAZC * 64]; B.N_RAZU = ringp[pn + RP_RAZU * 64];
                if (AUF) B.N_RAZV = ringp[(unsigned)kk * (RP_FIELDS * 64) + lane_it + RP_RAZV * 64];
                else { const double x = ringp[pn + RP_RAZV * 64]; B.N_RAZV = razv_delay; razv_delay = x; }
            };
            B.template step<PRE, decltype(midB), true, true>(T, ks, kv, q, bu_p, bv_p, bP_0, bm_0, ba_0, s11, s22, s12, bun, bvn, q >= ja - 1, q >= ja, pb1, pb2, mhistB, FB,
                   off2(max(q, row0)), c2s, off2(max(q + 1, row0)), off2(max(q - 1, row0)), midB, off2(max(q, row0)));
            fq = q; f11 = B.S11_0; f22 = B.S22_0; f12 = B.S12_0; ffirst = B.first; fsecond = B.second; fhave = true;
        } else {
        B.template step<PRE>(T, ks, kv, q, bu_p, bv_p, bP_0, bm_0, ba_0, s11, s22, s12, bun, bvn, q >= ja - 1, q >= ja, pb1, pb2, mhistB, FB);
        flush(q, B.S11_0, B.S22_0, B.S12_0, B.first, B.second, Idx<(CSI_PAIR_STORES & 7)>{}, Idx<AUF ? 1 : 0>{});
        }
        if ((CSI_PAIR_STORES & 7) != 7) {
            const unsigned so = (unsigned)((r - rstart) & 1) * (5 * 64) + (unsigned)lane;
            if (!(CSI_PAIR_STORES & 1)) { outr[so] = B.S11_0; outr[so + 64] = B.S22_0; outr[so + 128] = B.S12_0; }
            if (!(CSI_PAIR_STORES & 2)) outr[so + 192] = B.first;
            if (!(CSI_PAIR_STORES & 4)) outr[so + 256] = B.second;
        }
        if (write_diag) {
            if (((flags & L_RS) != 0) & (q >= rs_lo) & (q <= rs_hi)) {
                const unsigned ocq = offc(q), ofq = offf(q);
                const int yq = yimg(q);
                put(5, ocq, (unsigned)yq * sc, q <= HyW, dx, B.AL_0, q, yq);
                put(7, ofq, (unsigned)yq * sf, q <= HyW, dx, 0.5 * B.zf, q, yq);
                put(6, ocq, (unsigned)yq * sc, q <= HyW, dx, 0.5 * B.zc, q, yq);
                put(8, ocq, (unsigned)yq * sc, q <= HyW, dx, B.Dc * B.rDc, q, yq);
            }
        }
        B.shift(bu_p, bv_p, bm_0, ba_0);
        PROBE(pacc2);
    };
    for (;;) {
        bodyB(Idx<0>{});
        if (++r > rend) break;
        bodyB(Idx<1>{});
        if (++r > rend) break;
        bodyB(Idx<2>{});
        if (++r > rend) break;
    }
    if constexpr (FULL) {
        if (fhave) flush(fq, f11, f22, f12, ffirst, fsecond, Idx<(CSI_PAIR_STORES & 7)>{}, Idx<AUF ? 1 : 0>{});
    }
    __syncthreads();
    publish();
#define PSTAGE B
    PROBE_END(w * 2 + 1);
#undef PSTAGE
#undef peer_abort
}

template <bool UNI, bool AUF, bool WALLS, bool MASK, bool FORCE, bool FD, int CF, bool FULL = false, bool PEER = false, int EXTRA = 0, bool DLD = false>
__global__ void __launch_bounds__(128, (FULL || (FORCE && (EXTRA != 1 || !MASK) && CSI_PAIR_FRING)) ? CSI_PAIR_FULL_WAVES
                                       : (UNI && !(EXTRA == 1 && MASK)) ? CSI_PAIR_UNI_WAVES : CSI_PAIR_WAVES) k_pair(const FusedTable* __restrict__ table, int nstrips, int nchunks, int rows,
                                                              int blocks_per_xcd, int write_diag, unsigned long long seq) {
    constexpr bool FRING = FORCE && !FULL && (EXTRA != 1 || !MASK) && CSI_PAIR_FRING;
    constexpr bool PRE = CSI_PAIR_PRE && !MASK && !FULL && !FRING && !(CSI_PAIR_LDSC_NOPRE && !UNI && !(EXTRA == 1 && MASK) && (CSI_PAIR_LDSC != 0));
    constexpr int RING_FIELDS = FRING ? 10 + RF_FORCING : (PRE ? 13 : 10);
    __shared__ double ring[RING_ROWS * RING_FIELDS * 64];
    __shared__ double ringp[FULL ? RP_ROWS * RP_FIELDS * 64 : 1];
    __shared__ unsigned ringm[MASK ? RING_ROWS * 64 : 1];
    __shared__ double outr[(CSI_PAIR_STORES & 7) != 7 ? 2 * 5 * 64 : 1];
    __shared__ unsigned peer_abort_w;
#ifdef CSI_EXP_LDSPAD
    __shared__ double lds_pad[(FULL && FORCE) ? CSI_EXP_LDSPAD / 8 : 1];
    if (FULL && FORCE) { lds_pad[threadIdx.x] = 0.0; asm volatile("" :: "v"(lds_pad[threadIdx.x])); }
#endif
    constexpr bool LDSC = !UNI && !FULL && !(EXTRA == 1 && MASK) && (CSI_PAIR_LDSC != 0);
    __shared__ double ringc[LDSC ? 8 * FC_COUNT : 1];
    const int b = (int)blockIdx.x;
    int w = (b & 7) * blocks_per_xcd + (b >> 3);
    if (write_diag & 12) {
        typedef const __attribute__((address_space(4))) int* iptr_t;
        iptr_t act = (iptr_t)((tptr_t)table)->P[(write_diag & 8) ? FP_ACT_LIVE0 : FP_ACT_LIVE];
        const int live = act[0], per = (live + 7) >> 3, k = b >> 3, p = (b & 7) * per + k;
        if ((k >= per) | (p >= live)) return;
        w = act[2 + p];
    } else if (w >= nstrips * nchunks) return;
    if constexpr (PEER) {
        const int chunk = w / nstrips, strip = w - chunk * nstrips;
        tptr_t T = (tptr_t)table;
        const bool pw = strip < T->I[FI_PSET], pe = strip >= nstrips - T->I[FI_PSET + 1], ps = chunk < T->I[FI_PSET + 2],
                   pn = chunk >= nchunks - T->I[FI_PSET + 3];
        const unsigned pd = ((pw ? 1u : 0u) | (pe ? 2u : 0u) | (ps ? 4u : 0u) | (pn ? 8u : 0u) | ((ps & pw) ? 16u : 0u) | ((ps & pe) ? 32u : 0u) |
                             ((pn & pw) ? 64u : 0u) | ((pn & pe) ? 128u : 0u)) & (unsigned)T->I[FI_PMASK];
        if (__builtin_amdgcn_readfirstlane((int)pd) == 0) {
            pair_body<UNI, AUF, WALLS, MASK, FORCE, FD, CF, FULL, false, EXTRA, false>(table, w, nstrips, nchunks, rows, blocks_per_xcd, write_diag, seq, ring, ringm, outr, &peer_abort_w, ringp, ringc);
            return;
        }
    }
    pair_body<UNI, AUF, WALLS, MASK, FORCE, FD, CF, FULL, PEER, EXTRA, DLD>(table, w, nstrips, nchunks, rows, blocks_per_xcd, write_diag, seq, ring, ringm, outr, &peer_abort_w, ringp, ringc);
}

}

#if defined(CSI_PAIR_PROBE) && (!defined(CSI_PAIR_VARIANT) || CSI_PAIR_VARIANT == 0)
extern "C" int csi_debug_probe(unsigned long long* dst) {
    return (int)hipMemcpyFromSymbol(dst, HIP_SYMBOL(fused::g_probe), sizeof(unsigned long long) * 8192 * 16);
}
#endif
#if defined(CSI_PAIR_PROBE) && defined(CSI_PAIR_VARIANT) && CSI_PAIR_VARIANT >= 1
#define CSI_PROBE_NAME_(v) csi_debug_probe_v##v
#define CSI_PROBE_NAME(v) CSI_PROBE_NAME_(v)
extern "C" int CSI_PROBE_NAME(CSI_PAIR_VARIANT)(unsigned long long* dst) {
    return (int)hipMemcpyFromSymbol(dst, HIP_SYMBOL(fused::g_probe), sizeof(unsigned long long) * 8192 * 16);
}
#endif

#ifndef CSI_PAIR_VARIANT
#define CSI_PAIR_VARIANT 0
#endif
#if CSI_PAIR_VARIANT == 0
#define CSI_PAIR_NAME launch_fused_pair_plain
#define CSI_PAIR_FLAGS false, false, false, false
#elif CSI_PAIR_VARIANT == 1
#define CSI_PAIR_NAME launch_fused_pair_walls
#define CSI_PAIR_FLAGS true, false, false, false
#elif CSI_PAIR_VARIANT == 2
#define CSI_PAIR_NAME launch_fused_pair_mask
#define CSI_PAIR_FLAGS true, true, false, false
#elif CSI_PAIR_VARIANT == 3
#define CSI_PAIR_NAME launch_fused_pair_force
#define CSI_PAIR_FLAGS true, false, true, false
#elif CSI_PAIR_VARIANT == 4
#define CSI_PAIR_NAME launch_fused_pair_mask_force
#define CSI_PAIR_FLAGS true, true, true, false
#elif CSI_PAIR_VARIANT == 5
#define CSI_PAIR_NAME launch_fused_pair_force_fd
#define CSI_PAIR_FLAGS true, false, true, true
#elif CSI_PAIR_VARIANT == 6
#define CSI_PAIR_NAME launch_fused_pair_mask_force_fd
#define CSI_PAIR_FLAGS true, true, true, true
#elif CSI_PAIR_VARIANT == 7
#define CSI_PAIR_NAME launch_fused_pair_force_x
#define CSI_PAIR_FLAGS true, false, true, false
#define CSI_PAIR_EXTRA 1
#elif CSI_PAIR_VARIANT == 8
#define CSI_PAIR_NAME launch_fused_pair_mask_force_x
#define CSI_PAIR_FLAGS true, true, true, false
#define CSI_PAIR_EXTRA 1
#elif CSI_PAIR_VARIANT == 9
#define CSI_PAIR_NAME launch_fused_pair_force_w
#define CSI_PAIR_FLAGS true, false, true, false
#define CSI_PAIR_EXTRA 2
#else
#define CSI_PAIR_NAME launch_fused_pair_mask_force_w
#define CSI_PAIR_FLAGS true, true, true, false
#define CSI_PAIR_EXTRA 2
#endif
#ifndef CSI_PAIR_EXTRA
#define CSI_PAIR_EXTRA 0
#endif
void CSI_PAIR_NAME(const FusedTable* dev_table, int metric, bool a_ufirst, int common, int nstrips, int nchunks, int rows,
                   int write_diag, unsigned long long seq, hipStream_t s) {
    const int nblocks = nstrips * nchunks;
    const int per_xcd = (nblocks + 7) / 8;
    dim3 grid((unsigned)(per_xcd * 8)), block(128);
    const bool dld = (seq >> 63) != 0;
    seq &= ~(1ull << 63);
    (void)dld;
#if CSI_PAIR_VARIANT >= 1
#define CSI_LAUNCH_PAIR_(U, A, C, F) do { if (seq && dld) hipLaunchKernelGGL((fused::k_pair<U, A, CSI_PAIR_FLAGS, C, F, true, CSI_PAIR_EXTRA, true>), grid, block, 0, s, dev_table, nstrips, nchunks, rows, per_xcd, write_diag, seq); \
                                          else if (seq) hipLaunchKernelGGL((fused::k_pair<U, A, CSI_PAIR_FLAGS, C, F, true, CSI_PAIR_EXTRA>), grid, block, 0, s, dev_table, nstrips, nchunks, rows, per_xcd, write_diag, seq); \
                                          else hipLaunchKernelGGL((fused::k_pair<U, A, CSI_PAIR_FLAGS, C, F, false, CSI_PAIR_EXTRA>), grid, block, 0, s, dev_table, nstrips, nchunks, rows, per_xcd, write_diag, seq); } while (0)
#else
#define CSI_LAUNCH_PAIR_(U, A, C, F) do { if (seq) hipLaunchKernelGGL((fused::k_pair<U, A, CSI_PAIR_FLAGS, C, F, true, CSI_PAIR_EXTRA>), grid, block, 0, s, dev_table, nstrips, nchunks, rows, per_xcd, write_diag, seq); \
                                          else hipLaunchKernelGGL((fused::k_pair<U, A, CSI_PAIR_FLAGS, C, F, false, CSI_PAIR_EXTRA>), grid, block, 0, s, dev_table, nstrips, nchunks, rows, per_xcd, write_diag, seq); } while (0)
#endif
#if CSI_PAIR_VARIANT <= 2
#define CSI_LAUNCH_PAIR(U, A) do { if (common == 2) CSI_LAUNCH_PAIR_(U, A, 2, false); else if (common) CSI_LAUNCH_PAIR_(U, A, 1, false); else CSI_LAUNCH_PAIR_(U, A, 0, false); } while (0)
#else
#define CSI_LAUNCH_PAIR(U, A) do { (void)common; CSI_LAUNCH_PAIR_(U, A, 0, false); } while (0)
#endif
    if (metric == 2) {
#if CSI_PAIR_VARIANT >= 1 && CSI_PAIR_VARIANT <= 2
        if (common == 2) { if (a_ufirst) CSI_LAUNCH_PAIR_(false, true, 2, true); else CSI_LAUNCH_PAIR_(false, false, 2, true); }
        else { if (a_ufirst) CSI_LAUNCH_PAIR_(false, true, 0, true); else CSI_LAUNCH_PAIR_(false, false, 0, true); }
#elif CSI_PAIR_VARIANT >= 1
        if (a_ufirst) CSI_LAUNCH_PAIR_(false, true, 0, true); else CSI_LAUNCH_PAIR_(false, false, 0, true);
#endif
    } else if (metric == 0) { if (a_ufirst) CSI_LAUNCH_PAIR(true, true); else CSI_LAUNCH_PAIR(true, false); }
    else { if (a_ufirst) CSI_LAUNCH_PAIR(false, true); else CSI_LAUNCH_PAIR(false, false); }
#undef CSI_LAUNCH_PAIR
#undef CSI_LAUNCH_PAIR_
}

#if CSI_PAIR_VARIANT == 0
void launch_fused_pair_walls(const FusedTable*, int, bool, int, int, int, int, int, unsigned long long, hipStream_t);
void launch_fused_pair_mask(const FusedTable*, int, bool, int, int, int, int, int, unsigned long long, hipStream_t);
void launch_fused_pair_force(const FusedTable*, int, bool, int, int, int, int, int, unsigned long long, hipStream_t);
void launch_fused_pair_mask_force(const FusedTable*, int, bool, int, int, int, int, int, unsigned long long, hipStream_t);
void launch_fused_pair_force_fd(const FusedTable*, int, bool, int, int, int, int, int, unsigned long long, hipStream_t);
void launch_fused_pair_mask_force_fd(const FusedTable*, int, bool, int, int, int, int, int, unsigned long long, hipStream_t);
void launch_fused_pair_force_x(const FusedTable*, int, bool, int, int, int, int, int, unsigned long long, hipStream_t);
void launch_fused_pair_mask_force_x(const FusedTable*, int, bool, int, int, int, int, int, unsigned long long, hipStream_t);
void launch_fused_pair_force_w(const FusedTable*, int, bool, int, int, int, int, int, unsigned long long, hipStream_t);
void launch_fused_pair_mask_force_w(const FusedTable*, int, bool, int, int, int, int, int, unsigned long long, hipStream_t);
void launch_fused_pair(const FusedTable* dev_table, int metric, bool a_ufirst, bool walls, bool mask, bool force, bool free_drift, int extra,
                       int common, int nstrips, int nchunks, int rows, int write_diag, unsigned long long seq, hipStream_t s) {
    if (metric == 2) walls = true;
    if (extra == 2 && mask) launch_fused_pair_mask_force_w(dev_table, metric, a_ufirst, common, nstrips, nchunks, rows, write_diag, seq, s);
    else if (extra == 2) launch_fused_pair_force_w(dev_table, metric, a_ufirst, common, nstrips, nchunks, rows, write_diag, seq, s);
    else if (extra && mask) launch_fused_pair_mask_force_x(dev_table, metric, a_ufirst, common, nstrips, nchunks, rows, write_diag, seq, s);
    else if (extra) launch_fused_pair_force_x(dev_table, metric, a_ufirst, common, nstrips, nchunks, rows, write_diag, seq, s);
    else if (free_drift && mask) launch_fused_pair_mask_force_fd(dev_table, metric, a_ufirst, common, nstrips, nchunks, rows, write_diag, seq, s);
    else if (free_drift) launch_fused_pair_force_fd(dev_table, metric, a_ufirst, common, nstrips, nchunks, rows, write_diag, seq, s);
    else if (force && mask) launch_fused_pair_mask_force(dev_table, metric, a_ufirst, common, nstrips, nchunks, rows, write_diag, seq, s);
    else if (force) launch_fused_pair_force(dev_table, metric, a_ufirst, common, nstrips, nchunks, rows, write_diag, seq, s);
    else if (mask) launch_fused_pair_mask(dev_table, metric, a_ufirst, common, nstrips, nchunks, rows, write_diag, seq, s);
    else if (walls) launch_fused_pair_walls(dev_table, metric, a_ufirst, common, nstrips, nchunks, rows, write_diag, seq, s);
    else launch_fused_pair_plain(dev_table, metric, a_ufirst, common, nstrips, nchunks, rows, write_diag, seq, s);
}
#endif

}
```

climaseaice.jl_amd/csrc/evp_pair_stage.h:

```cpp
#pragma once
#include "evp_fused_common.h"

namespace csi {
namespace fused {

constexpr int P_LO = 4, P_HI = 59, P_W = P_HI - P_LO + 1;

struct Forcing {
    double t_tau_u, t_we_u, t_wb_u, b_tau_u, b_we_u, b_wb_u, t_tau_v, t_we_v, t_wb_v, b_tau_v, b_we_v, b_wb_v;
    double fd_u, fd_v;
    bool fd;
    double xc_u, xd_u, xc_v, xd_v;
    int extra;
};

struct RowIn { double u_p, v_p, P_0, h_0, a_0, s11, s22, s12, un_m, vn_x; unsigned mk; double ck; };

__device__ __forceinline__ unsigned left_bits(unsigned x) { return (unsigned)__builtin_amdgcn_mov_dpp((int)x, 0x138, 0xf, 0xf, true); }

__device__ __forceinline__ void full_cell(tptr_t T, unsigned o, unsigned s2, double u_0, double v_0, double v_p, double& e11, double& e22, int rcd = 0) {
    const double dyu = c2at(T, C2_DYU + rcd, o), dxv_s = c2at(T, C2_DXV + rcd, o), dxv_n = c2at(T, C2_DXV + rcd, o + s2);
    const double Uy_w = dyu * u_0, Ur_w = fm::rcp(dyu) * u_0;
    const double Vx_s = dxv_s * v_0, Vr_s = fm::rcp(dxv_s) * v_0;
    const double Vx_n = dxv_n * v_p, Vr_n = fm::rcp(dxv_n) * v_p;
    fm::full_strain_cell(from_right(Uy_w), Uy_w, Vx_n, Vx_s, from_right(Ur_w), Ur_w, Vr_n, Vr_s,
                         c2at(T, C2_DYC2 + rcd, o), c2at(T, C2_DXC2 + rcd, o), c2at(T, C2_RAZC + rcd, o), e11, e22);
}
__device__ __forceinline__ double full_corner(tptr_t T, unsigned o, unsigned s2, double u_n, double u_s, double v_e, int rcd = 0) {
    const double Ux_n = c2at(T, C2_RDXU + rcd, o) * u_n, Ux_s = c2at(T, C2_RDXU + rcd, o - s2) * u_s;
    const double Vy_e = c2at(T, C2_RDYV + rcd, o) * v_e;
    return fm::full_strain_corner(Ux_n, Ux_s, Vy_e, from_left(Vy_e), c2at(T, C2_DXF2 + rcd, o), c2at(T, C2_DYF2 + rcd, o), c2at(T, C2_RAZF + rcd, o));
}

template <bool UNI, bool UFIRST, bool MASK, bool TIGHT = false, int CF = 0, bool FULL = false, bool HOLDK = true>
struct Stage {
    double u_m, u_0, v_m, v_0, Xv_m, Xv_0;
    double a_mm, a_m, m_mm, m_m;
    double XP_m, Xm_m, Xa_m, Xe11_m, Xe22_m, Ye12_0, e12_0;
    double XAL_m, XS11L_m, XW, Wprev;
    double XS22L_m;
    double DXV_0, RDXV_0, RDYV_0, RDXU_0, DXF2_0, DYF2_0, RAZF_0;
    double DXV_m, RDXV_m, RDYV_m, RDXU_m, DXF2_m, DYF2_m, DYU_m, RDYU_m, DYC2_m, DXC2_m, DXC2_mm;
    double DXV_p, RDXV_p, RDYV_p, RDXU_p, DXF2_p, DYF2_p, RAZF_p, DYU_0, RDYU_0, DYC2_0, DXC2_0;
#ifndef CSI_FULL_HOISTP
#define CSI_FULL_HOISTP 1
#endif
#if CSI_FULL_HOISTP >= 1
    unsigned long c2p[12];
    int rcd_ = 0;
    __device__ __forceinline__ void hoist_planes(tptr_t T, int rcd = 0) {
        rcd_ = rcd;
#pragma unroll
        for (int k = 0; k < 12; ++k) c2p[k] = T->P[FP_C2_0 + k + rcd];
    }
    __device__ __forceinline__ double c2m(tptr_t, int which, unsigned off) const { return ldg_keep(c2p[which], off); }
#else
    int rcd_ = 0;
    __device__ __forceinline__ void hoist_planes(tptr_t, int rcd = 0) { rcd_ = rcd; }
    __device__ __forceinline__ double c2m(tptr_t T, int which, unsigned off) const { return c2at(T, which + rcd_, off); }
#endif
    __device__ __forceinline__ unsigned long f2u(tptr_t T) const { return T->P[FP_F2U + rcd_]; }
    __device__ __forceinline__ unsigned long f2v(tptr_t T) const { return T->P[FP_F2V + rcd_]; }
    double RAZC_0, RAZU_m, RAZV_x, FU_m, FV_x;

#ifndef CSI_PAIR_VK
#define CSI_PAIR_VK 1
#endif
    static constexpr bool VKC = UNI && !FULL && HOLDK && (CSI_PAIR_VK != 0);
    double VK_E, VK_FN, VK_FS, VK_FU, VK_Q2N, VK_K, VK_FV, VK_BRHO;
    __device__ __forceinline__ void hoist_uniform(tptr_t T) {
        if constexpr (VKC) {
            VK_E = T->K[FK_PCOEF0 + FC_E]; VK_FN = T->K[FK_PCOEF0 + FC_FN]; VK_FS = T->K[FK_PCOEF0 + FC_FS]; VK_FU = T->K[FK_PCOEF0 + FC_FU];
            VK_Q2N = T->K[FK_PCOEF0 + FC_Q2N]; VK_K = T->K[FK_PCOEF0 + FC_K]; VK_FV = T->K[FK_PCOEF0 + FC_FV]; VK_BRHO = T->K[FK_BOT_RHOCD];
            asm volatile("" : "+v"(VK_E), "+v"(VK_FN), "+v"(VK_FS), "+v"(VK_FU), "+v"(VK_Q2N), "+v"(VK_K), "+v"(VK_FV), "+v"(VK_BRHO));
        }
    }
#ifndef CSI_PAIR_LDSC
#define CSI_PAIR_LDSC 0
#endif
    static constexpr bool LDSC = !UNI && !FULL && HOLDK && (CSI_PAIR_LDSC != 0);
    const double* lc = nullptr;
    __device__ __forceinline__ double pc(tptr_t T, int which, int j) const {
        if constexpr (LDSC) return lc[(unsigned)(j & 7) * FC_COUNT + which]; else return pcoef<UNI>(T, which, j);
    }
    __device__ __forceinline__ double vk(tptr_t T, int which, int j, double held) const { if constexpr (VKC) return held; else return pc(T, which, j); }
    __device__ __forceinline__ double brho(tptr_t T) const { if constexpr (VKC) return VK_BRHO; else return T->K[FK_BOT_RHOCD]; }

    double N_DXV, N_RDYV, N_RDXU, N_DXF2, N_DYF2, N_RAZF, N_DYU, N_DYC2, N_DXC2, N_RAZC;
    double N_RAZU, N_RAZV, N_FU, N_FV;
    __device__ __forceinline__ void full_prefetch_vel(tptr_t T, unsigned on, unsigned om) {
        N_RAZU = c2m(T, C2_RAZU, om); N_RAZV = c2m(T, C2_RAZV, UFIRST ? om : on);
        N_FU = 0.0; N_FV = 0.0;
        if (T->I[FI_FKIND] == 2) { N_FU = ldg(f2u(T), om); N_FV = ldg(f2v(T), UFIRST ? om : on); }
    }
    __device__ __forceinline__ void full_prefetch_f(tptr_t T, unsigned on, unsigned om) {
        N_FU = 0.0; N_FV = 0.0;
        if (T->I[FI_FKIND] == 2) { N_FU = ldg(f2u(T), om); N_FV = ldg(f2v(T), UFIRST ? om : on); }
    }
    __device__ __forceinline__ void full_prefetch(tptr_t T, unsigned on, unsigned s2) {
        N_DXV = c2m(T, C2_DXV, on + s2); N_RDYV = c2m(T, C2_RDYV, on + s2); N_RDXU = c2m(T, C2_RDXU, on + s2);
        N_DXF2 = c2m(T, C2_DXF2, on + s2); N_DYF2 = c2m(T, C2_DYF2, on + s2); N_RAZF = c2m(T, C2_RAZF, on + s2);
        N_DYU = c2m(T, C2_DYU, on); N_DYC2 = c2m(T, C2_DYC2, on); N_DXC2 = c2m(T, C2_DXC2, on); N_RAZC = c2m(T, C2_RAZC, on);
    }
    __device__ __forceinline__ void full_init(tptr_t T, unsigned o, unsigned om, unsigned s2) {
        full_prefetch(T, o, s2);
        DXV_0 = c2m(T, C2_DXV, o); RDXV_0 = fm::rcp(DXV_0); RDYV_0 = c2m(T, C2_RDYV, o); RDXU_0 = c2m(T, C2_RDXU, o);
        DXF2_0 = c2m(T, C2_DXF2, o); DYF2_0 = c2m(T, C2_DYF2, o); RAZF_0 = c2m(T, C2_RAZF, o);
        DXV_m = DXV_0; RDXV_m = RDXV_0; RDYV_m = RDYV_0; RDXU_m = RDXU_0; DXF2_m = DXF2_0; DYF2_m = DYF2_0;
        DYU_m = c2m(T, C2_DYU, o); RDYU_m = fm::rcp(DYU_m); DYC2_m = c2m(T, C2_DYC2, o); DXC2_m = c2m(T, C2_DXC2, o); DXC2_mm = DXC2_m;
    }
    double S11_mm, S22_mm, S12_mm, AL_mm, S11_m, S22_m, S12_m, AL_m;
#ifdef CSI_PAIR_PROBE
    unsigned long long sp0 = 0, sp1 = 0, sp2 = 0, sp3 = 0, spt = 0;
#define SPROBE_START do { __builtin_amdgcn_sched_barrier(0); spt = __builtin_readcyclecounter(); __builtin_amdgcn_sched_barrier(0); } while (0)
#define SPROBE(acc) do { __builtin_amdgcn_sched_barrier(0); const unsigned long long t_ = __builtin_readcyclecounter(); \
                         __builtin_amdgcn_sched_barrier(0); acc += t_ - spt; spt = t_; } while (0)
#else
#define SPROBE_START do { } while (0)
#define SPROBE(acc) do { } while (0)
#endif
    double S11_0, S22_0, S12_0, AL_0, zc, zf, Dc, rDc, first, second;
    double Xv_p, Xa_0, Xm_0, e12_p, XW_next;
    double Pf_0, rmc_0, rmf_0;

    struct NoMid { __device__ __forceinline__ void operator()() const {} };
    template <bool PRE = false, class MID = NoMid, bool ALLPRE = false, bool PLR = false>
    __device__ __forceinline__ void step(tptr_t T, const fm::StressConst& ks_in, const fm::VelConst& kv_in, int r,
                                         double u_p, double v_p, double P_0, double m_0, double a_0,
                                         double s11, double s22, double s12, double un_m, double vn_x,
                                         bool do_stress, bool do_vel, bool per_first, bool per_second, unsigned mh,
                                         const Forcing& F, unsigned o2 = 0u, unsigned s2 = 0u, unsigned o2n = 0u, unsigned o2m = 0u, MID mid = MID(), unsigned o2nm = 0u) {
        SPROBE_START;
        Xa_0 = fm::sum2(from_left(a_0), a_0);
        Xv_p = fm::sum2(from_left(v_p), v_p);
        double e11_0, e22_0;
        if constexpr (FULL) {
            DXV_p = N_DXV; RDXV_p = fm::rcp(DXV_p); RDYV_p = N_RDYV; RDXU_p = N_RDXU;
            DXF2_p = N_DXF2; DYF2_p = N_DYF2; RAZF_p = N_RAZF;
            DYU_0 = N_DYU; RDYU_0 = fm::rcp(DYU_0); DYC2_0 = N_DYC2; DXC2_0 = N_DXC2;
            RAZC_0 = N_RAZC;
            if constexpr (ALLPRE) {
                RAZU_m = N_RAZU; RAZV_x = N_RAZV; FU_m = N_FU; FV_x = N_FV;
            } else if (do_vel) {
                RAZU_m = c2m(T, C2_RAZU, o2m); RAZV_x = c2m(T, C2_RAZV, UFIRST ? o2m : o2);
                if (T->I[FI_FKIND] == 2) { FU_m = ldg(f2u(T), o2m); FV_x = ldg(f2v(T), UFIRST ? o2m : o2); }
            }
            const double Uy_w = DYU_0 * u_0, Ur_w = RDYU_0 * u_0;
            fm::full_strain_cell(from_right(Uy_w), Uy_w, DXV_p * v_p, DXV_0 * v_0, from_right(Ur_w), Ur_w, RDXV_p * v_p, RDXV_0 * v_0,
                                 DYC2_0, DXC2_0, RAZC_0, e11_0, e22_0);
            const double Vy_e = RDYV_p * v_p;
            e12_p = fm::full_strain_corner8(RDXU_p * u_p, RDXU_0 * u_0, Vy_e, from_left(Vy_e), DXF2_p, DYF2_p, RAZF_p);
        } else {
        fm::strain_cell<UNI>(pc(T, FC_A, r), pc(T, FC_BN, r), pc(T, FC_BS, r), pc(T, FC_CN, r),
                        pc(T, FC_CS, r), from_right(u_0), u_0, v_p, v_0, e11_0, e22_0);
        e12_p = fm::strain_corner<UNI>(pc(T, FC_SN, r + 1), pc(T, FC_SS, r + 1), pc(T, FC_SV, r + 1),
                                  u_p, u_0, v_p, from_left(v_p));
        }
        {
            const double Xe11_0 = fm::sum2(from_left(e11_0), e11_0), Xe22_0 = fm::sum2(from_left(e22_0), e22_0);
            const double Ye12_p = fm::sum2(e12_p, from_right(e12_p));
            Xm_0 = fm::sum2(from_left(m_0), m_0);
            const double e11f = fm::sum2(Xe11_m, Xe11_0);
            const double e22f = fm::sum2(Xe22_m, Xe22_0);
            const double e12c = 0.0625 * fm::sum2(Ye12_0, Ye12_p);
            const double mf = fm::sum2(Xm_m, Xm_0);
            if constexpr (!PRE) {
                const double XP_0 = fm::sum2(from_left(P_0), P_0);
                Pf_0 = fm::sum2(XP_m, XP_0);
                XP_m = XP_0;
                rmc_0 = fm::rcp(m_0); rmf_0 = fm::rcp(mf);
            }
            const double Pf = Pf_0;
            Xe11_m = Xe11_0; Xe22_m = Xe22_0; Ye12_0 = Ye12_p;
            SPROBE(sp0);
            if (do_stress) {
                fm::StressConst ks = ks_in;
                if (CF) ks.pressure_kind = 0;
                if (TIGHT) {
                    asm volatile("" : "+s"(T));
                    ks.em2 = T->K[FK_EM2]; ks.Dmin = T->K[FK_DMIN]; ks.Dmin2 = T->K[FK_DMIN2]; ks.amin2 = T->K[FK_AMIN2];
                    ks.amax2 = T->K[FK_AMAX2]; ks.hk1 = T->K[FK_HK1]; ks.pressure_kind = T->I[FI_PRESSURE_KIND];
                    ks.em2_8 = T->K[FK_PK_EM2_8]; ks.Dmin2_16 = T->K[FK_PK_DMIN2_16];
                }
                double kc, kf;
                if constexpr (FULL) { kc = T->K[FK_CA_DT] * RAZC_0; kf = T->K[FK_PK_CA_DT4] * RAZF_0; }
                else { kc = UNI ? T->K[FK_HKC] : T->K[FK_CA_DT] * pc(T, FC_RAZC, r); kf = UNI ? T->K[FK_PK_HKF4] : T->K[FK_PK_CA_DT4] * pc(T, FC_RAZF, r); }
                const fm::StressOut o = fm::stress_update_s(ks, e11_0, e22_0, e12_0, e11f, e22f, e12c, P_0, Pf, m_0, mf, rmc_0, rmf_0, kc, kf, s11, s22, s12);
                S11_0 = o.s11; S22_0 = o.s22; S12_0 = o.s12; AL_0 = o.alpha; zc = o.zc2; zf = o.zf2; Dc = o.xc; rDc = o.rDc;
            }
        }
        double d11_0 = S11_0, d22_0 = S22_0, d12_0 = S12_0, d11_m = S11_m, d22_m = S22_m, d12_m = S12_m, d11_mm = S11_mm, d22_mm = S22_mm;
        double d11_mL = XS11L_m, d22_mL = XS22L_m;
        if (MASK) {
            const unsigned m0 = mh & 3u, m1 = (mh >> 2) & 3u, m2 = (mh >> 4) & 3u;
            const bool pcc_0 = m0 == 1u, pcc_m = m1 == 1u, pcc_mm = m2 == 1u;
            unsigned c0 = m0 | m1, c1 = m1 | m2;
            c0 |= left_bits(c0); c1 |= left_bits(c1);
            const bool pff_0 = (c0 & 3u) == 1u, pff_m = (c1 & 3u) == 1u;
            d11_0 = pcc_0 ? 0.0 : S11_0; d22_0 = pcc_0 ? 0.0 : S22_0;
            d11_m = pcc_m ? 0.0 : S11_m; d22_m = pcc_m ? 0.0 : S22_m;
            d11_mm = pcc_mm ? 0.0 : S11_mm; d22_mm = pcc_mm ? 0.0 : S22_mm;
            d12_0 = pff_0 ? 0.0 : S12_0; d12_m = pff_m ? 0.0 : S12_m;
            d11_mL = from_left(d11_m);
            if constexpr (FULL) d22_mL = from_left(d22_m);
            const bool ia_0 = (m0 & 1u) != 0, ia_m = (m1 & 1u) != 0, ia_mm = (m2 & 1u) != 0;
            const bool ia_mL = (left_bits(m1) & 1u) != 0;
            const bool per_u = ia_m | ia_mL;
            per_first = UFIRST ? per_u : (ia_0 | ia_m);
            per_second = UFIRST ? (ia_m | ia_mm) : per_u;
        }
        auto div1_full = [&]() __attribute__((always_inline)) {
            const double S_e = d11_m + d22_m, T_e = DYC2_m * (d11_m - d22_m);
            const double S_w = MASK ? from_left(S_e) : d11_mL + d22_mL;
            const double T_w = MASK ? from_left(T_e) : from_left(DYC2_m) * (d11_mL - d22_mL);
            return fm::full_div1_x2(DYU_m, RDYU_m, RDXU_m, RAZU_m, S_e, S_w, T_e, T_w, DXF2_0 * d12_0, DXF2_m * d12_m);
        };
        auto div2_full = [&](bool low) __attribute__((always_inline)) {
            if (low) {
                const double Zw = DYF2_m * d12_m;
                return fm::full_div2_x2(DXV_m, RDXV_m, RDYV_m, RAZV_x, d11_m + d22_m, d11_mm + d22_mm,
                                     DXC2_m * (d11_m - d22_m), DXC2_mm * (d11_mm - d22_mm), from_right(Zw), Zw);
            }
            const double Zw = DYF2_0 * d12_0;
            return fm::full_div2_x2(DXV_0, RDXV_0, RDYV_0, RAZV_x, d11_0 + d22_0, d11_m + d22_m,
                                 DXC2_0 * (d11_0 - d22_0), DXC2_m * (d11_m - d22_m), from_right(Zw), Zw);
        };
        auto f_full = [&](int which_row, int which_plane, unsigned o, int j) __attribute__((always_inline)) {
            const int kind = T->I[FI_FKIND];
            if (kind == 2) return which_plane == FP_F2U ? FU_m : FV_x;
            if (kind == 1) { typedef const __attribute__((address_space(4))) double* vptr_t; return ((vptr_t)T->P[which_row])[j]; }
            return T->K[FK_FCOR];
        };
        SPROBE(sp1);
        if constexpr (FULL) {
            __builtin_amdgcn_sched_barrier(0);
            if constexpr (!PLR) full_prefetch(T, o2n, s2);
            if constexpr (ALLPRE) { if constexpr (PLR) full_prefetch_f(T, o2n, o2nm); else full_prefetch_vel(T, o2n, o2nm); }
            mid();
            __builtin_amdgcn_sched_barrier(0);
        }
        SPROBE(sp2);
        fm::VelConst kv = kv_in;
        if (TIGHT) {
            asm volatile("" : "+s"(T));
            kv.dt = T->K[FK_DT2]; kv.rdt = T->K[FK_RDT]; kv.min_mass = T->K[FK_MIN_MASS2]; kv.min_conc = T->K[FK_MIN_CONC2];
        }
        if (!do_vel) {
            XW_next = XW;
        } else if (UFIRST) {
            const int j = r - 1;
            double W_0;
            {
                const double vbar = fm::quarter(Xv_m, Xv_0);
                double div;
                if constexpr (FULL) div = div1_full();
                else div = fm::div1(vk(T, FC_E, j, VK_E), vk(T, FC_FN, j, VK_FN), vk(T, FC_FS, j, VK_FS),
                                            d11_m, d11_mL, d12_0, d12_m);
                double ext, imt, exb, imb;
                if (CF) { ext = F.t_tau_u; imt = 0.0; } else fm::ext_stress(T->I[FI_TOP_KIND], F.t_tau_u, T->K[FK_TOP_RHOCD], F.t_we_u, F.t_wb_u, u_m, vbar, ext, imt);
                if (CF == 2) fm::ext_stress_rest(brho(T), u_m, vbar, exb, imb);
                else fm::ext_stress(CF ? 3 : T->I[FI_BOT_KIND], F.b_tau_u, brho(T), F.b_we_u, F.b_wb_u, u_m, vbar, exb, imb);
                double cor;
                if constexpr (FULL) cor = f_full(FP_FROW_U, FP_F2U, o2 - s2, j) * vbar;
                else cor = vk(T, FC_FU, j, VK_FU) * vbar;
                if (F.extra & 1) cor += F.xc_u;
                if (F.extra & 2) div = fm::fma_(2.0, F.xd_u, div);
                W_0 = F.fd ? fm::vel_update_sum_fd(kv, u_m, un_m, Xm_m, Xa_m, XAL_m, div, cor, ext, imt, exb, imb, per_first, F.fd_u)
                           : fm::vel_update_sum(kv, u_m, un_m, Xm_m, Xa_m, XAL_m, div, cor, ext, imt, exb, imb, per_first);
            }
            const double XW_0 = fm::sum2(W_0, from_right(W_0));
            {
                const double ubar = fm::quarter(XW, XW_0);
                double div;
                if constexpr (FULL) div = div2_full(true);
                else div = fm::div2<UNI>(pc(T, FC_Q1N, j), vk(T, FC_Q2N, j, VK_Q2N), pc(T, FC_Q1S, j),
                                            pc(T, FC_Q2S, j), vk(T, FC_K, j, VK_K),
                                            d11_m, d22_m, d11_mm, d22_mm, from_right(d12_m), d12_m);
                double ext, imt, exb, imb;
                if (CF) { ext = F.t_tau_v; imt = 0.0; } else fm::ext_stress(T->I[FI_TOP_KIND], F.t_tau_v, T->K[FK_TOP_RHOCD], F.t_we_v, F.t_wb_v, v_m, ubar, ext, imt);
                if (CF == 2) fm::ext_stress_rest(brho(T), v_m, ubar, exb, imb);
                else fm::ext_stress(CF ? 3 : T->I[FI_BOT_KIND], F.b_tau_v, brho(T), F.b_we_v, F.b_wb_v, v_m, ubar, exb, imb);
                double cor;
                if constexpr (FULL) cor = -f_full(FP_FROW_V, FP_F2V, o2 - s2, j) * ubar;
                else cor = -vk(T, FC_FV, j, VK_FV) * ubar;
                if (F.extra & 1) cor += F.xc_v;
                if (F.extra & 2) div = fm::fma_(2.0, F.xd_v, div);
                second = F.fd ? fm::vel_update_sum_fd(kv, v_m, vn_x, m_mm + m_m, a_mm + a_m, AL_mm + AL_m, div, cor, ext, imt, exb, imb, per_second, F.fd_v)
                              : fm::vel_update_sum(kv, v_m, vn_x, m_mm + m_m, a_mm + a_m, AL_mm + AL_m, div, cor, ext, imt, exb, imb, per_second);
            }
            first = W_0;
            XW_next = XW_0;
        } else {
            double W_0;
            {
                const double ubar = fm::avg4(u_m, from_right(u_m), u_0, from_right(u_0));
                double div;
                if constexpr (FULL) div = div2_full(false);
                else div = fm::div2<UNI>(pc(T, FC_Q1N, r), vk(T, FC_Q2N, r, VK_Q2N), pc(T, FC_Q1S, r),
                                            pc(T, FC_Q2S, r), vk(T, FC_K, r, VK_K),
                                            d11_0, d22_0, d11_m, d22_m, from_right(d12_0), d12_0);
                double ext, imt, exb, imb;
                if (CF) { ext = F.t_tau_v; imt = 0.0; } else fm::ext_stress(T->I[FI_TOP_KIND], F.t_tau_v, T->K[FK_TOP_RHOCD], F.t_we_v, F.t_wb_v, v_0, ubar, ext, imt);
                if (CF == 2) fm::ext_stress_rest(brho(T), v_0, ubar, exb, imb);
                else fm::ext_stress(CF ? 3 : T->I[FI_BOT_KIND], F.b_tau_v, brho(T), F.b_we_v, F.b_wb_v, v_0, ubar, exb, imb);
                double cor;
                if constexpr (FULL) cor = -f_full(FP_FROW_V, FP_F2V, o2, r) * ubar;
                else cor = -vk(T, FC_FV, r, VK_FV) * ubar;
                if (F.extra & 1) cor += F.xc_v;
                if (F.extra & 2) div = fm::fma_(2.0, F.xd_v, div);
                W_0 = F.fd ? fm::vel_update_sum_fd(kv, v_0, vn_x, m_m + m_0, a_m + a_0, AL_m + AL_0, div, cor, ext, imt, exb, imb, per_first, F.fd_v)
                           : fm::vel_update_sum(kv, v_0, vn_x, m_m + m_0, a_m + a_0, AL_m + AL_0, div, cor, ext, imt, exb, imb, per_first);
            }
            const double XW_0 = fm::sum2(from_left(W_0), W_0);
            {
                const int j = r - 1;
                const double vbar = fm::quarter(XW, XW_0);
                double div;
                if constexpr (FULL) div = div1_full();
                else div = fm::div1(vk(T, FC_E, j, VK_E), vk(T, FC_FN, j, VK_FN), vk(T, FC_FS, j, VK_FS),
                                            d11_m, d11_mL, d12_0, d12_m);
                double ext, imt, exb, imb;
                if (CF) { ext = F.t_tau_u; imt = 0.0; } else fm::ext_stress(T->I[FI_TOP_KIND], F.t_tau_u, T->K[FK_TOP_RHOCD], F.t_we_u, F.t_wb_u, u_m, vbar, ext, imt);
                if (CF == 2) fm::ext_stress_rest(brho(T), u_m, vbar, exb, imb);
                else fm::ext_stress(CF ? 3 : T->I[FI_BOT_KIND], F.b_tau_u, brho(T), F.b_we_u, F.b_wb_u, u_m, vbar, exb, imb);
                double cor;
                if constexpr (FULL) cor = f_full(FP_FROW_U, FP_F2U, o2 - s2, j) * vbar;
                else cor = vk(T, FC_FU, j, VK_FU) * vbar;
                if (F.extra & 1) cor += F.xc_u;
                if (F.extra & 2) div = fm::fma_(2.0, F.xd_u, div);
                second = F.fd ? fm::vel_update_sum_fd(kv, u_m, un_m, Xm_m, Xa_m, XAL_m, div, cor, ext, imt, exb, imb, per_second, F.fd_u)
                              : fm::vel_update_sum(kv, u_m, un_m, Xm_m, Xa_m, XAL_m, div, cor, ext, imt, exb, imb, per_second);
            }
            first = W_0;
            XW_next = XW_0;
        }
        SPROBE(sp3);
    }

    __device__ __forceinline__ void shift(double u_p, double v_p, double m_0, double a_0) {
        u_m = u_0; u_0 = u_p; v_m = v_0; v_0 = v_p;
        Xv_m = Xv_0; Xv_0 = Xv_p;
        a_mm = a_m; a_m = a_0; m_mm = m_m; m_m = m_0;
        Xm_m = Xm_0; Xa_m = Xa_0;
        e12_0 = e12_p;
        S11_mm = S11_m; S22_mm = S22_m; S12_mm = S12_m; AL_mm = AL_m;
        S11_m = S11_0; S22_m = S22_0; S12_m = S12_0; AL_m = AL_0;
        XAL_m = fm::sum2(from_left(AL_0), AL_0); XS11L_m = from_left(S11_0);
        if constexpr (FULL) {
            XS22L_m = from_left(S22_0);
            DXV_m = DXV_0; RDXV_m = RDXV_0; RDYV_m = RDYV_0; RDXU_m = RDXU_0; DXF2_m = DXF2_0; DYF2_m = DYF2_0;
            DXV_0 = DXV_p; RDXV_0 = RDXV_p; RDYV_0 = RDYV_p; RDXU_0 = RDXU_p; DXF2_0 = DXF2_p; DYF2_0 = DYF2_p; RAZF_0 = RAZF_p;
            DYU_m = DYU_0; RDYU_m = RDYU_0; DYC2_m = DYC2_0; DXC2_mm = DXC2_m; DXC2_m = DXC2_0;
        }
        XW = XW_next;
        Wprev = first;
    }
};


}
}
```

Before: 71.06 billion cell-updates/s.

## Pass precomputed reciprocals and neighbor loads through the producer-consumer ring

In the uniform, no-mask, no-forcing fast path, the producer now loads left/right neighbor values (u, v, P, a) directly from global memory rather than getting them through cross-lane shuffles. It also computes the velocity reciprocal mass, the concentration ratio, the activity flags and the stress positivity flags once, then publishes them via extra ring fields and a byte mask. The consumer stage reads these instead of recomputing rcp and the comparisons. This aims to cut DPP/shuffle traffic and duplicate reciprocal math, at the cost of more global loads, ring LDS space and register pressure.

```diff
diff --git a/climaseaice.jl_amd/csrc/evp_fast_math.h b/climaseaice.jl_amd/csrc/evp_fast_math.h
--- a/climaseaice.jl_amd/csrc/evp_fast_math.h
+++ b/climaseaice.jl_amd/csrc/evp_fast_math.h
@@ -104,10 +104,11 @@
     return o;
 }
 
-__device__ __forceinline__ StressOut stress_update_s(const StressConst& k, double e11c, double e22c, double E12f,
-                                                     double S11f, double S22f, double y2, double Pc, double XP,
-                                                     double mc, double M4, double rmc, double rM4, double hkc, double hkf4,
-                                                     double s11, double s22, double s12) {
+template <class PC, class PF>
+__device__ __forceinline__ StressOut stress_update_sp(const StressConst& k, double e11c, double e22c, double E12f,
+                                                      double S11f, double S22f, double y2, double Pc, double XP,
+                                                      PC mc_pos, PF M4_pos, double rmc, double rM4, double hkc, double hkf4,
+                                                      double s11, double s22, double s12) {
     StressOut o;
     const double dc = e11c + e22c, DF = S11f + S22f;
     const double tc = e11c - e22c, TF = S11f - S22f;
@@ -128,13 +129,19 @@
     double gc, rgc, gf, rgf;
     sqrt_rsqrt(g2c, gc, rgc);
     sqrt_rsqrt(g2f, gf, rgf);
-    const double wc = (mc > 0) ? rgc : 0.0, wf = (M4 > 0) ? rgf : 0.0;
+    const double wc = mc_pos() ? rgc : 0.0, wf = M4_pos() ? rgf : 0.0;
     o.s11 = fma_(s11n - s11, wc, s11);
     o.s22 = fma_(s22n - s22, wc, s22);
     o.s12 = fma_(s12n - s12, wf, s12);
     o.alpha = gc;
     o.zc2 = zc2; o.zf2 = zf2; o.xc = xc; o.rDc = rDc;
     return o;
+}
+__device__ __forceinline__ StressOut stress_update_s(const StressConst& k, double e11c, double e22c, double E12f,
+                                                     double S11f, double S22f, double y2, double Pc, double XP,
+                                                     double mc, double M4, double rmc, double rM4, double hkc, double hkf4,
+                                                     double s11, double s22, double s12) {
+    return stress_update_sp(k, e11c, e22c, E12f, S11f, S22f, y2, Pc, XP, [&]() __attribute__((always_inline)) { return mc > 0; }, [&]() __attribute__((always_inline)) { return M4 > 0; }, rmc, rM4, hkc, hkf4, s11, s22, s12);
 }
 
 __device__ __forceinline__ StressOut stress_update(const StressConst& k, double e11c, double e22c, double e12f,
@@ -199,25 +206,37 @@
     return vel_update_avg_fd(k, w, wn, avg2(m_a, m_b), avg2(a_a, a_b), avg2(al_a, al_b), div, cor, ext, imt, exb, imb, peripheral, wf);
 }
 
+template <class ACT>
+__device__ __forceinline__ double vel_update_sum_r(const VelConst& k2, double w, double wn, double rm2, double rai, ACT active_ice, double al2,
+                                                   double div2, double cor, double ext, double imt, double exb, double imb, bool peripheral) {
+    const double G = fma_(wn - w, k2.rdt, fma_(div2, rm2, fma_(exb - ext, rai, cor)));
+    const double tau_i = (imb - imt) * rai;
+    const double wD = fma_(k2.dt, G, al2 * w) * rcp(fma_(k2.dt, tau_i, al2));
+    double res = active_ice() ? wD : 0.0;
+    return peripheral ? 0.0 : res;
+}
+template <class ACT, class MAR>
+__device__ __forceinline__ double vel_update_sum_fd_r(const VelConst& k2, double w, double wn, double rm2, double rai, ACT active_ice, MAR marginal,
+                                                      double al2, double div2, double cor, double ext, double imt, double exb, double imb,
+                                                      bool peripheral, double wf) {
+    const double wD = vel_update_sum_r(k2, w, wn, rm2, rai, active_ice, al2, div2, cor, ext, imt, exb, imb, false);
+    const bool act = active_ice(), mar = marginal();
+    const double res = act ? wD : (mar ? wf : 0.0);
+    return peripheral ? 0.0 : res;
+}
 __device__ __forceinline__ double vel_update_sum(const VelConst& k2, double w, double wn, double m2, double a2, double al2,
                                                  double div2, double cor, double ext, double imt, double exb, double imb, bool peripheral) {
     const double rm2 = rcp(m2);
     const double rai = rm2 * a2;
-    const double G = fma_(wn - w, k2.rdt, fma_(div2, rm2, fma_(exb - ext, rai, cor)));
-    const double tau_i = (imb - imt) * rai;
-    const double wD = fma_(k2.dt, G, al2 * w) * rcp(fma_(k2.dt, tau_i, al2));
-    const bool active_ice = (m2 >= k2.min_mass) & (a2 >= k2.min_conc);
-    double res = active_ice ? wD : 0.0;
-    return peripheral ? 0.0 : res;
+    return vel_update_sum_r(k2, w, wn, rm2, rai, [&]() __attribute__((always_inline)) { return (m2 >= k2.min_mass) & (a2 >= k2.min_conc); }, al2, div2, cor, ext, imt, exb, imb, peripheral);
 }
 __device__ __forceinline__ double vel_update_sum_fd(const VelConst& k2, double w, double wn, double m2, double a2, double al2,
                                                     double div2, double cor, double ext, double imt, double exb, double imb,
                                                     bool peripheral, double wf) {
-    const double wD = vel_update_sum(k2, w, wn, m2, a2, al2, div2, cor, ext, imt, exb, imb, false);
-    const bool active_ice = (m2 >= k2.min_mass) & (a2 >= k2.min_conc);
-    const bool marginal = (m2 > 2.0 * CSI_EPS64) & (a2 > 2.0 * CSI_EPS64);
-    const double res = active_ice ? wD : (marginal ? wf : 0.0);
-    return peripheral ? 0.0 : res;
+    const double rm2 = rcp(m2);
+    const double rai = rm2 * a2;
+    return vel_update_sum_fd_r(k2, w, wn, rm2, rai, [&]() __attribute__((always_inline)) { return (m2 >= k2.min_mass) & (a2 >= k2.min_conc); },
+                               [&]() __attribute__((always_inline)) { return (m2 > 2.0 * CSI_EPS64) & (a2 > 2.0 * CSI_EPS64); }, al2, div2, cor, ext, imt, exb, imb, peripheral, wf);
 }
 
 __device__ __forceinline__ double div1(double E, double Fn, double Fs, double s11_0, double s11_m, double s12_p, double s12_0) {
diff --git a/climaseaice.jl_amd/csrc/evp_fused2.hip b/climaseaice.jl_amd/csrc/evp_fused2.hip
--- a/climaseaice.jl_amd/csrc/evp_fused2.hip
+++ b/climaseaice.jl_amd/csrc/evp_fused2.hip
@@ -29,6 +29,12 @@
 #endif
 #ifndef CSI_PAIR_SKIPB
 #define CSI_PAIR_SKIPB 0
+#endif
+#ifndef CSI_PAIR_NBR
+#define CSI_PAIR_NBR 1
+#endif
+#ifndef CSI_PAIR_VINV
+#define CSI_PAIR_VINV 1
 #endif
 #ifndef CSI_PAIR_PD
 #define CSI_PAIR_PD 1
@@ -58,6 +64,7 @@
 
 constexpr int RING_ROWS = 4;
 enum : int { RF_S11 = 0, RF_S22, RF_S12, RF_U, RF_V, RF_P, RF_M, RF_A, RF_UN, RF_VN, RF_PF, RF_RMC, RF_RMF };
+enum : int { RF_RM2U = RF_M, RF_RAIU = RF_A, RF_RM2V = 13, RF_RAIV = 14 };
 #ifndef CSI_PAIR_LDSC_NOPRE
 #define CSI_PAIR_LDSC_NOPRE 1
 #endif
@@ -80,7 +87,11 @@
     constexpr bool LDSC = !UNI && !FULL && !(EXTRA == 1 && MASK) && (CSI_PAIR_LDSC != 0);
     constexpr bool FRING = FORCE && !FULL && (EXTRA != 1 || !MASK) && CSI_PAIR_FRING;
     constexpr bool PRE = CSI_PAIR_PRE && !MASK && !FULL && !FRING && !(CSI_PAIR_LDSC_NOPRE && !UNI && !(EXTRA == 1 && MASK) && (CSI_PAIR_LDSC != 0));
-    constexpr int RING_FIELDS = FRING ? 10 + RF_FORCING : (PRE ? 13 : 10);
+    constexpr bool DIETF = UNI && !WALLS && !MASK && !FORCE && !FD && !FULL && EXTRA == 0;
+    constexpr bool NBR = DIETF && (CSI_PAIR_NBR != 0), VINV = DIETF && PRE && (CSI_PAIR_VINV != 0);
+    constexpr int DIET = (NBR ? D_NBR : 0) | (VINV ? D_VINV : 0);
+    constexpr int RING_FIELDS = FRING ? 10 + RF_FORCING : (VINV ? 15 : (PRE ? 13 : 10));
+    static_assert(RF_U >= 1 && RF_V + 1 < RING_FIELDS, "the consumer reads u, v at lane -+ 1: one element beyond the field's row, inside the ring");
 #define peer_abort (*peer_abort_p)
     const int b = (int)blockIdx.x;
 #ifndef CSI_EXP_ROLESWAP
@@ -95,6 +106,7 @@
 
     int ja, jb, rstart, rend;
     unsigned loff, sc, sf;
+    unsigned loffl = 0, loffr = 0;
     unsigned lm = 0, sm = 0;
     int i;
     unsigned flags;
@@ -119,6 +131,10 @@
         }
         const int ic = min(max(i, 1 - Hx), Nx + Hx);
         loff = (unsigned)(ic - (1 - Hx)) * 8u;
+        if constexpr (NBR) {
+            loffl = (unsigned)(min(max(i - 1, 1 - Hx), Nx + Hx) - (1 - Hx)) * 8u;
+            loffr = (unsigned)(min(max(i + 1, 1 - Hx), Nx + Hx) - (1 - Hx)) * 8u;
+        }
         row0 = 1 - Hy;
         const bool own = (lane >= P_LO) & (lane <= P_HI) & (i <= T->I[FI_DEC + 1]);
         flags = 0;
@@ -432,7 +448,7 @@
 
     if (!consumer) {
         PROBE_DECL;
-        Stage<UNI, AUF, MASK, FORCE, CF, FULL, !(EXTRA == 1 && MASK)> A;
+        Stage<UNI, AUF, MASK, FORCE, CF, FULL, !(EXTRA == 1 && MASK), DIET> A;
         A.lc = ringc;
         const int cjmin = LDSC ? T->I[FI_COEF_JMIN] : 0, cjmax = LDSC ? T->I[FI_COEF_JMAX] : 0;
         const unsigned ck_lane = (unsigned)min(lane, FC_COUNT - 1) * 8u;
@@ -444,6 +460,9 @@
 #endif
         auto alias_row = [&](int j) __attribute__((always_inline)) { return CSI_EXP_RINGALIAS ? min(max(j, ja + 1), max(jb - 1, ja + 1)) : j; };
         unsigned oc = offc(alias_row(rstart)), of = offf(alias_row(rstart)), om = MASK ? offm(rstart) : 0u;
+        unsigned ocl = oc - loff + loffl, ofrp = of - loff + loffr + sf;
+        auto pin = [&]() __attribute__((always_inline)) { if constexpr (NBR) asm volatile("" : "+v"(oc), "+v"(of), "+v"(ocl), "+v"(ofrp)); };
+        pin();
         {
             const double rho0 = T->K[FK_RHO];
             A.u_m = ldg(T->P[FP_U_IN], of - sf); A.v_m = ldg(T->P[FP_V_IN], oc - sc);
@@ -456,6 +475,8 @@
             A.Xa_m = fm::sum2(from_left(A.a_m), A.a_m);
             A.Xv_m = fm::sum2(from_left(A.v_m), A.v_m);
             A.Xv_0 = fm::sum2(from_left(A.v_0), A.v_0);
+            if constexpr (NBR) { A.uR_m = from_right(A.u_m); A.uR_0 = from_right(A.u_0); }
+            if constexpr (VINV) { A.rm2_u = 0.0; A.rai_u = 0.0; A.rm2_v = 0.0; A.rai_v = 0.0; A.act_u = false; A.act_v = false; A.pos_c = false; A.pos_f = false; }
             double e11_m, e22_m;
             const int jm = rstart - 1;
             A.hoist_uniform(T);
@@ -479,6 +500,10 @@
         }
 #pragma unroll
         for (int q = 0; q < RING_ROWS * RING_FIELDS; ++q) ring[q * 64 + lane] = 0.0;
+        if constexpr (VINV) {
+#pragma unroll
+            for (int q = 0; q < RING_ROWS; ++q) ringm[q * 64 + lane] = 0u;
+        }
         if constexpr (FULL) {
 #pragma unroll
             for (int q = 0; q < RP_ROWS * RP_FIELDS; ++q) ringp[q * 64 + lane] = 1.0;
@@ -492,6 +517,7 @@
             ringm[(unsigned)((-1) & (RING_ROWS - 1)) * 64 + (unsigned)lane] = mhist & 3u;
         }
         RowIn R[3];
+        Nbr RN[3];
 #ifndef CSI_FULL_HOISTP
 #define CSI_FULL_HOISTP 1
 #endif
@@ -503,7 +529,7 @@
                             hA = HIN ? T->P[FP_A] : 0ul, h11 = HIN ? T->P[FP_S11_IN] : 0ul, h22 = HIN ? T->P[FP_S22_IN] : 0ul, h12 = HIN ? T->P[FP_S12_IN] : 0ul,
                             hUN = HIN ? T->P[FP_UN] : 0ul, hVN = HIN ? T->P[FP_VN] : 0ul;
         int rnext = rstart;
-        auto load_row = [&](RowIn& Q) __attribute__((always_inline)) {
+        auto load_row = [&](RowIn& Q, Nbr& QN) __attribute__((always_inline)) {
             if constexpr (HIN) {
                 Q.u_p = ldg(hU, of + sf); Q.v_p = ldg(hV, oc + sc);
                 Q.P_0 = ldg(hP, oc); Q.h_0 = ldg(hH, oc); Q.a_0 = ldg(hA, oc);
@@ -515,13 +541,18 @@
             Q.s11 = ldg(T->P[FP_S11_IN], oc); Q.s22 = ldg(T->P[FP_S22_IN], oc); Q.s12 = ldg(T->P[FP_S12_IN], of);
             Q.un_m = ldg(T->P[FP_UN], of - sf); Q.vn_x = ldg(T->P[FP_VN], AUF ? oc - sc : oc);
             }
+            if constexpr (NBR) {
+                QN.u_rp = ldg(T->P[FP_U_IN], ofrp); QN.v_lp = ldg(T->P[FP_V_IN], ocl + sc);
+                QN.P_l = ldg(T->P[FP_P], ocl); QN.a_l = ldg(T->P[FP_A], ocl);
+            }
             Q.mk = MASK ? ldub(T->P[FP_MASK], om) : 1u;
             if constexpr (LDSC) Q.ck = ldg(coef_row_base(rnext + 2), ck_lane);
         };
         auto advance = [&]() __attribute__((always_inline)) {
             const bool more = rnext < rend;
-            if (CSI_EXP_RINGALIAS) { rnext += more ? 1 : 0; oc = offc(alias_row(rnext)); of = offf(alias_row(rnext)); return; }
+            if (CSI_EXP_RINGALIAS) { rnext += more ? 1 : 0; oc = offc(alias_row(rnext)); of = offf(alias_row(rnext)); ocl = oc - loff + loffl; ofrp = of - loff + loffr + sf; return; }
             oc += more ? sc : 0u; of += more ? sf : 0u;
+            if constexpr (NBR) { ocl += more ? sc : 0u; ofrp += more ? sf : 0u; pin(); }
             if (MASK) om += more ? sm : 0u;
             rnext += more ? 1 : 0;
         };
@@ -549,7 +580,7 @@
             if (FORCE) arrays(FA, offf(r - 1), AUF ? offc(r - 1) : offc(r));
             if constexpr (!FULL) {
                 advance();
-                load_row(R[(k + CSI_PAIR_PD) % 3]);
+                load_row(R[(k + CSI_PAIR_PD) % 3], RN[(k + CSI_PAIR_PD) % 3]);
             }
             flush(r - 4, o11, o22, o12, ofirst, osecond, Idx<PW>{}, Idx<AUF ? 1 : 0>{});
             fm::StressConst ks; stress_consts(ks);
@@ -563,9 +594,13 @@
             }
             if constexpr (FULL) {
                 static_assert(CSI_PAIR_PD == 1, "the per-point-metric producer prefetches one row ahead");
-                auto mid = [&]() __attribute__((always_inline)) { advance(); load_row(R[(k + 1) % 3]); };
+                auto mid = [&]() __attribute__((always_inline)) { advance(); load_row(R[(k + 1) % 3], RN[(k + 1) % 3]); };
                 A.template step<false>(T, ks, kv, r, C.u_p, C.v_p, C.P_0, m_0, C.a_0, C.s11, C.s22, C.s12, C.un_m, C.vn_x, true, r > rstart, pa1, pa2, mhist, FA,
                                        off2(r), c2s, off2(min(r + 1, rend)), off2(max(r - 1, row0)), mid);
+            } else if constexpr (NBR) {
+                const Nbr& nb = RN[k];
+                A.step(T, ks, kv, r, C.u_p, C.v_p, C.P_0, m_0, C.a_0, C.s11, C.s22, C.s12, C.un_m, C.vn_x, true, r > rstart, pa1, pa2, mhist, FA,
+                       0u, 0u, 0u, 0u, typename decltype(A)::NoMid(), 0u, nb);
             } else
             A.step(T, ks, kv, r, C.u_p, C.v_p, C.P_0, m_0, C.a_0, C.s11, C.s22, C.s12, C.un_m, C.vn_x, true, r > rstart, pa1, pa2, mhist, FA);
             {
@@ -576,7 +611,13 @@
                 if (single) {
                     ring[s0 + RF_P * 64] = A.AL_0; ring[s0 + RF_M * 64] = 0.5 * A.zf; ring[s0 + RF_A * 64] = 0.5 * A.zc; ring[s0 + RF_VN * 64] = A.Dc * A.rDc;
                 } else {
-                ring[s0 + RF_P * 64] = C.P_0; ring[s0 + RF_M * 64] = m_0; ring[s0 + RF_A * 64] = C.a_0;
+                ring[s0 + RF_P * 64] = C.P_0;
+                if constexpr (VINV) {
+                    ring[s1 + RF_RM2U * 64] = inv_tag(A.rm2_u, A.act_u); ring[s1 + RF_RAIU * 64] = A.rai_u;
+                    ring[(AUF ? s1 : s0) + RF_RM2V * 64] = inv_tag(A.rm2_v, A.act_v); ring[(AUF ? s1 : s0) + RF_RAIV * 64] = A.rai_v;
+                    unsigned char* pb = (unsigned char*)(ringm + ((unsigned)((r - rstart) & (RING_ROWS - 1)) * 64 + lane_it));
+                    pb[0] = A.pos_c ? 1 : 0; pb[1] = A.pos_f ? 1 : 0;
+                } else { ring[s0 + RF_M * 64] = m_0; ring[s0 + RF_A * 64] = C.a_0; }
                 if (PRE) { ring[s0 + RF_PF * 64] = A.Pf_0; ring[s0 + RF_RMC * 64] = A.rmc_0; ring[s0 + RF_RMF * 64] = A.rmf_0; }
                 ring[s1 + RF_UN * 64] = C.un_m; ring[(AUF ? s1 : s0) + RF_VN * 64] = C.vn_x;
                 }
@@ -617,10 +658,10 @@
                 if (lane < FC_COUNT) ringc[(unsigned)((rstart + d) & 7) * FC_COUNT + (unsigned)lane] = v;
             }
         }
-        load_row(R[0]);
+        load_row(R[0], RN[0]);
         if (CSI_PAIR_PD == 2) {
             advance();
-            load_row(R[1]);
+            load_row(R[1], RN[1]);
         }
         for (;;) {
             body(Idx<0>{});
@@ -692,9 +733,10 @@
     }
 
     PROBE_DECL;
-    Stage<UNI, !AUF, MASK, FORCE, CF, FULL, !(EXTRA == 1 && MASK)> B;
+    Stage<UNI, !AUF, MASK, FORCE, CF, FULL, !(EXTRA == 1 && MASK), DIET> B;
     B.lc = ringc;
     B.u_m = 0; B.u_0 = 0; B.v_m = 0; B.v_0 = 0; B.Xv_m = 0; B.Xv_0 = 0;
+    if constexpr (NBR) { B.uR_m = 0; B.uR_0 = 0; }
     B.a_mm = 0; B.a_m = 0; B.m_mm = 0; B.m_m = 0;
     B.XP_m = 0; B.Xm_m = 0; B.Xa_m = 0; B.Xe11_m = 0; B.Xe22_m = 0; B.Ye12_0 = 0; B.e12_0 = 0;
     B.XAL_m = 0; B.XS11L_m = 0; B.XS22L_m = 0; B.XW = 0; B.Wprev = 0;
@@ -713,6 +755,7 @@
     const int rlo = rstart - 1;
     unsigned mhistB = 0xffffffffu;
     double vn_delay = 0.0;
+    double rm2v_delay = 0.0, raiv_delay = 0.0;
     double razv_delay = 1.0;
     double fvd_tau = 0.0, fvd_we = 0.0, fvd_wb = 0.0, fvd_fd = 0.0;
     int r = rstart;
@@ -729,7 +772,19 @@
         const unsigned s1 = rslot(r - 1), s2 = rslot(r - 2), s3 = rslot(r - 3);
         double bu_p = ring[s1 + RF_U * 64], bv_p = ring[s1 + RF_V * 64];
         const double s11 = ring[s2 + RF_S11 * 64], s22 = ring[s2 + RF_S22 * 64], s12 = ring[s2 + RF_S12 * 64];
-        const double bP_0 = ring[s2 + RF_P * 64], bm_0 = ring[s2 + RF_M * 64], ba_0 = ring[s2 + RF_A * 64];
+        const double bP_0 = ring[s2 + RF_P * 64], bm_0 = VINV ? 0.0 : ring[s2 + RF_M * 64], ba_0 = VINV ? 0.0 : ring[s2 + RF_A * 64];
+        Nbr nbB{0.0, 0.0, 0.0, 0.0};
+        if constexpr (NBR) {
+            nbB.u_rp = ring[s1 + RF_U * 64 + 1]; nbB.v_lp = ring[s1 + RF_V * 64 - 1];
+        }
+        if constexpr (VINV) {
+            B.rm2_u = ring[s3 + RF_RM2U * 64]; B.rai_u = ring[s3 + RF_RAIU * 64];
+            const double rv = ring[s2 + RF_RM2V * 64], av = ring[s2 + RF_RAIV * 64];
+            const unsigned char* pb = (const unsigned char*)(ringm + ((unsigned)((r - 2 - rstart) & (RING_ROWS - 1)) * 64 + lane_it));
+            B.pos_c = pb[0] != 0; B.pos_f = pb[1] != 0;
+            if (AUF) { B.rm2_v = rv; B.rai_v = av; }
+            else { B.rm2_v = rm2v_delay; B.rai_v = raiv_delay; rm2v_delay = rv; raiv_delay = av; }
+        }
         if (PRE) { B.Pf_0 = ring[s2 + RF_PF * 64]; B.rmc_0 = ring[s2 + RF_RMC * 64]; B.rmf_0 = ring[s2 + RF_RMF * 64]; }
         const double bun = ring[s3 + RF_UN * 64], vn_new = ring[s2 + RF_VN * 64];
         const double bvn = AUF ? vn_new : vn_delay;
@@ -799,6 +854,10 @@
             B.template step<PRE, decltype(midB), true, true>(T, ks, kv, q, bu_p, bv_p, bP_0, bm_0, ba_0, s11, s22, s12, bun, bvn, q >= ja - 1, q >= ja, pb1, pb2, mhistB, FB,
                    off2(max(q, row0)), c2s, off2(max(q + 1, row0)), off2(max(q - 1, row0)), midB, off2(max(q, row0)));
             fq = q; f11 = B.S11_0; f22 = B.S22_0; f12 = B.S12_0; ffirst = B.first; fsecond = B.second; fhave = true;
+        } else if constexpr (DIET != 0) {
+        B.template step<PRE>(T, ks, kv, q, bu_p, bv_p, bP_0, bm_0, ba_0, s11, s22, s12, bun, bvn, q >= ja - 1, q >= ja, pb1, pb2, mhistB, FB,
+                             0u, 0u, 0u, 0u, typename decltype(B)::NoMid(), 0u, nbB);
+        flush(q, B.S11_0, B.S22_0, B.S12_0, B.first, B.second, Idx<(CSI_PAIR_STORES & 7)>{}, Idx<AUF ? 1 : 0>{});
         } else {
         B.template step<PRE>(T, ks, kv, q, bu_p, bv_p, bP_0, bm_0, ba_0, s11, s22, s12, bun, bvn, q >= ja - 1, q >= ja, pb1, pb2, mhistB, FB);
         flush(q, B.S11_0, B.S22_0, B.S12_0, B.first, B.second, Idx<(CSI_PAIR_STORES & 7)>{}, Idx<AUF ? 1 : 0>{});
@@ -819,7 +878,7 @@
                 put(8, ocq, (unsigned)yq * sc, q <= HyW, dx, B.Dc * B.rDc, q, yq);
             }
         }
-        B.shift(bu_p, bv_p, bm_0, ba_0);
+        B.template shift<VINV>(bu_p, bv_p, bm_0, ba_0);
         PROBE(pacc2);
     };
     for (;;) {
@@ -847,10 +906,11 @@
                                                               int blocks_per_xcd, int write_diag, unsigned long long seq) {
     constexpr bool FRING = FORCE && !FULL && (EXTRA != 1 || !MASK) && CSI_PAIR_FRING;
     constexpr bool PRE = CSI_PAIR_PRE && !MASK && !FULL && !FRING && !(CSI_PAIR_LDSC_NOPRE && !UNI && !(EXTRA == 1 && MASK) && (CSI_PAIR_LDSC != 0));
-    constexpr int RING_FIELDS = FRING ? 10 + RF_FORCING : (PRE ? 13 : 10);
+    constexpr bool VINV = UNI && !WALLS && !MASK && !FORCE && !FD && !FULL && EXTRA == 0 && PRE && (CSI_PAIR_VINV != 0);
+    constexpr int RING_FIELDS = FRING ? 10 + RF_FORCING : (VINV ? 15 : (PRE ? 13 : 10));
     __shared__ double ring[RING_ROWS * RING_FIELDS * 64];
     __shared__ double ringp[FULL ? RP_ROWS * RP_FIELDS * 64 : 1];
-    __shared__ unsigned ringm[MASK ? RING_ROWS * 64 : 1];
+    __shared__ unsigned ringm[(MASK || VINV) ? RING_ROWS * 64 : 1];
     __shared__ double outr[(CSI_PAIR_STORES & 7) != 7 ? 2 * 5 * 64 : 1];
     __shared__ unsigned peer_abort_w;
 #ifdef CSI_EXP_LDSPAD
diff --git a/climaseaice.jl_amd/csrc/evp_pair_stage.h b/climaseaice.jl_amd/csrc/evp_pair_stage.h
--- a/climaseaice.jl_amd/csrc/evp_pair_stage.h
+++ b/climaseaice.jl_amd/csrc/evp_pair_stage.h
@@ -15,6 +15,11 @@
 };
 
 struct RowIn { double u_p, v_p, P_0, h_0, a_0, s11, s22, s12, un_m, vn_x; unsigned mk; double ck; };
+
+enum : int { D_NBR = 1, D_VINV = 2 };
+__device__ __forceinline__ double inv_tag(double rm2, bool active) { return __hiloint2double(active ? __double2hiint(rm2) : -1, __double2loint(rm2)); }
+__device__ __forceinline__ bool inv_active(double rm2) { return __double2hiint(rm2) >= 0; }
+struct Nbr { double a_l, P_l, v_lp, u_rp; };
 
 __device__ __forceinline__ unsigned left_bits(unsigned x) { return (unsigned)__builtin_amdgcn_mov_dpp((int)x, 0x138, 0xf, 0xf, true); }
 
@@ -32,9 +37,14 @@
     return fm::full_strain_corner(Ux_n, Ux_s, Vy_e, from_left(Vy_e), c2at(T, C2_DXF2 + rcd, o), c2at(T, C2_DYF2 + rcd, o), c2at(T, C2_RAZF + rcd, o));
 }
 
-template <bool UNI, bool UFIRST, bool MASK, bool TIGHT = false, int CF = 0, bool FULL = false, bool HOLDK = true>
+template <bool UNI, bool UFIRST, bool MASK, bool TIGHT = false, int CF = 0, bool FULL = false, bool HOLDK = true, int DIET = 0>
 struct Stage {
+    static constexpr bool NBR = (DIET & D_NBR) != 0, VINV = (DIET & D_VINV) != 0;
+    static_assert(DIET == 0 || (UNI && !MASK && !TIGHT && !FULL), "the diet is the uniform plain family's");
     double u_m, u_0, v_m, v_0, Xv_m, Xv_0;
+    double uR_m, uR_0;
+    double rm2_u, rai_u, rm2_v, rai_v;
+    bool act_u, act_v;
     double a_mm, a_m, m_mm, m_m;
     double XP_m, Xm_m, Xa_m, Xe11_m, Xe22_m, Ye12_0, e12_0;
     double XAL_m, XS11L_m, XW, Wprev;
@@ -120,7 +130,8 @@
 #define SPROBE(acc) do { } while (0)
 #endif
     double S11_0, S22_0, S12_0, AL_0, zc, zf, Dc, rDc, first, second;
-    double Xv_p, Xa_0, Xm_0, e12_p, XW_next;
+    double Xv_p, Xa_0, Xm_0, e12_p, XW_next, uR_p;
+    bool pos_c, pos_f;
     double Pf_0, rmc_0, rmf_0;
 
     struct NoMid { __device__ __forceinline__ void operator()() const {} };
@@ -129,10 +140,14 @@
                                          double u_p, double v_p, double P_0, double m_0, double a_0,
                                          double s11, double s22, double s12, double un_m, double vn_x,
                                          bool do_stress, bool do_vel, bool per_first, bool per_second, unsigned mh,
-                                         const Forcing& F, unsigned o2 = 0u, unsigned s2 = 0u, unsigned o2n = 0u, unsigned o2m = 0u, MID mid = MID(), unsigned o2nm = 0u) {
+                                         const Forcing& F, unsigned o2 = 0u, unsigned s2 = 0u, unsigned o2n = 0u, unsigned o2m = 0u, MID mid = MID(), unsigned o2nm = 0u,
+                                         const Nbr& nb = Nbr{0.0, 0.0, 0.0, 0.0}) {
         SPROBE_START;
-        Xa_0 = fm::sum2(from_left(a_0), a_0);
-        Xv_p = fm::sum2(from_left(v_p), v_p);
+        constexpr bool TAKE = VINV && PRE;
+        auto vL_p = [&]() __attribute__((always_inline)) { return NBR ? nb.v_lp : from_left(v_p); };
+        if constexpr (NBR) uR_p = nb.u_rp;
+        if constexpr (!TAKE) Xa_0 = fm::sum2(NBR ? nb.a_l : from_left(a_0), a_0);
+        Xv_p = fm::sum2(vL_p(), v_p);
         double e11_0, e22_0;
         if constexpr (FULL) {
             DXV_p = N_DXV; RDXV_p = fm::rcp(DXV_p); RDYV_p = N_RDYV; RDXU_p = N_RDXU;
@@ -152,20 +167,21 @@
             e12_p = fm::full_strain_corner8(RDXU_p * u_p, RDXU_0 * u_0, Vy_e, from_left(Vy_e), DXF2_p, DYF2_p, RAZF_p);
         } else {
         fm::strain_cell<UNI>(pc(T, FC_A, r), pc(T, FC_BN, r), pc(T, FC_BS, r), pc(T, FC_CN, r),
-                        pc(T, FC_CS, r), from_right(u_0), u_0, v_p, v_0, e11_0, e22_0);
+                        pc(T, FC_CS, r), NBR ? uR_0 : from_right(u_0), u_0, v_p, v_0, e11_0, e22_0);
         e12_p = fm::strain_corner<UNI>(pc(T, FC_SN, r + 1), pc(T, FC_SS, r + 1), pc(T, FC_SV, r + 1),
-                                  u_p, u_0, v_p, from_left(v_p));
+                                  u_p, u_0, v_p, vL_p());
         }
         {
             const double Xe11_0 = fm::sum2(from_left(e11_0), e11_0), Xe22_0 = fm::sum2(from_left(e22_0), e22_0);
             const double Ye12_p = fm::sum2(e12_p, from_right(e12_p));
-            Xm_0 = fm::sum2(from_left(m_0), m_0);
+            if constexpr (!TAKE) Xm_0 = fm::sum2(from_left(m_0), m_0);
             const double e11f = fm::sum2(Xe11_m, Xe11_0);
             const double e22f = fm::sum2(Xe22_m, Xe22_0);
             const double e12c = 0.0625 * fm::sum2(Ye12_0, Ye12_p);
-            const double mf = fm::sum2(Xm_m, Xm_0);
+            double mf = 0.0;
+            if constexpr (!TAKE) mf = fm::sum2(Xm_m, Xm_0);
             if constexpr (!PRE) {
-                const double XP_0 = fm::sum2(from_left(P_0), P_0);
+                const double XP_0 = fm::sum2(NBR ? nb.P_l : from_left(P_0), P_0);
                 Pf_0 = fm::sum2(XP_m, XP_0);
                 XP_m = XP_0;
                 rmc_0 = fm::rcp(m_0); rmf_0 = fm::rcp(mf);
@@ -185,7 +201,13 @@
                 double kc, kf;
                 if constexpr (FULL) { kc = T->K[FK_CA_DT] * RAZC_0; kf = T->K[FK_PK_CA_DT4] * RAZF_0; }
                 else { kc = UNI ? T->K[FK_HKC] : T->K[FK_CA_DT] * pc(T, FC_RAZC, r); kf = UNI ? T->K[FK_PK_HKF4] : T->K[FK_PK_CA_DT4] * pc(T, FC_RAZF, r); }
-                const fm::StressOut o = fm::stress_update_s(ks, e11_0, e22_0, e12_0, e11f, e22f, e12c, P_0, Pf, m_0, mf, rmc_0, rmf_0, kc, kf, s11, s22, s12);
+                fm::StressOut o;
+                if constexpr (VINV) {
+                    const bool mc_pos = TAKE ? pos_c : m_0 > 0, M4_pos = TAKE ? pos_f : mf > 0;
+                    if constexpr (!TAKE) { pos_c = mc_pos; pos_f = M4_pos; }
+                    o = fm::stress_update_sp(ks, e11_0, e22_0, e12_0, e11f, e22f, e12c, P_0, Pf, [&]() __attribute__((always_inline)) { return mc_pos; }, [&]() __attribute__((always_inline)) { return M4_pos; }, rmc_0, rmf_0, kc, kf, s11, s22, s12);
+                } else
+                o = fm::stress_update_s(ks, e11_0, e22_0, e12_0, e11f, e22f, e12c, P_0, Pf, m_0, mf, rmc_0, rmf_0, kc, kf, s11, s22, s12);
                 S11_0 = o.s11; S22_0 = o.s22; S12_0 = o.s12; AL_0 = o.alpha; zc = o.zc2; zf = o.zf2; Dc = o.xc; rDc = o.rDc;
             }
         }
@@ -245,6 +267,28 @@
             asm volatile("" : "+s"(T));
             kv.dt = T->K[FK_DT2]; kv.rdt = T->K[FK_RDT]; kv.min_mass = T->K[FK_MIN_MASS2]; kv.min_conc = T->K[FK_MIN_CONC2];
         }
+        auto upd_u = [&](double w, double wn, double m2, double a2, double al2, double div, double cor, double ext, double imt, double exb, double imb,
+                         bool per, double fdw) __attribute__((always_inline)) {
+            if constexpr (VINV) {
+                bool act;
+                if constexpr (TAKE) act = inv_active(rm2_u);
+                else { rm2_u = fm::rcp(m2); rai_u = rm2_u * a2; act = (m2 >= kv.min_mass) & (a2 >= kv.min_conc); act_u = act; }
+                return fm::vel_update_sum_r(kv, w, wn, rm2_u, rai_u, [&]() __attribute__((always_inline)) { return act; }, al2, div, cor, ext, imt, exb, imb, per);
+            } else
+            return F.fd ? fm::vel_update_sum_fd(kv, w, wn, m2, a2, al2, div, cor, ext, imt, exb, imb, per, fdw)
+                        : fm::vel_update_sum(kv, w, wn, m2, a2, al2, div, cor, ext, imt, exb, imb, per);
+        };
+        auto upd_v = [&](double w, double wn, double m2, double a2, double al2, double div, double cor, double ext, double imt, double exb, double imb,
+                         bool per, double fdw) __attribute__((always_inline)) {
+            if constexpr (VINV) {
+                bool act;
+                if constexpr (TAKE) act = inv_active(rm2_v);
+                else { rm2_v = fm::rcp(m2); rai_v = rm2_v * a2; act = (m2 >= kv.min_mass) & (a2 >= kv.min_conc); act_v = act; }
+                return fm::vel_update_sum_r(kv, w, wn, rm2_v, rai_v, [&]() __attribute__((always_inline)) { return act; }, al2, div, cor, ext, imt, exb, imb, per);
+            } else
+            return F.fd ? fm::vel_update_sum_fd(kv, w, wn, m2, a2, al2, div, cor, ext, imt, exb, imb, per, fdw)
+                        : fm::vel_update_sum(kv, w, wn, m2, a2, al2, div, cor, ext, imt, exb, imb, per);
+        };
         if (!do_vel) {
             XW_next = XW;
         } else if (UFIRST) {
@@ -265,8 +309,7 @@
                 else cor = vk(T, FC_FU, j, VK_FU) * vbar;
                 if (F.extra & 1) cor += F.xc_u;
                 if (F.extra & 2) div = fm::fma_(2.0, F.xd_u, div);
-                W_0 = F.fd ? fm::vel_update_sum_fd(kv, u_m, un_m, Xm_m, Xa_m, XAL_m, div, cor, ext, imt, exb, imb, per_first, F.fd_u)
-                           : fm::vel_update_sum(kv, u_m, un_m, Xm_m, Xa_m, XAL_m, div, cor, ext, imt, exb, imb, per_first);
+                W_0 = upd_u(u_m, un_m, Xm_m, Xa_m, XAL_m, div, cor, ext, imt, exb, imb, per_first, F.fd_u);
             }
             const double XW_0 = fm::sum2(W_0, from_right(W_0));
             {
@@ -285,15 +328,14 @@
                 else cor = -vk(T, FC_FV, j, VK_FV) * ubar;
                 if (F.extra & 1) cor += F.xc_v;
                 if (F.extra & 2) div = fm::fma_(2.0, F.xd_v, div);
-                second = F.fd ? fm::vel_update_sum_fd(kv, v_m, vn_x, m_mm + m_m, a_mm + a_m, AL_mm + AL_m, div, cor, ext, imt, exb, imb, per_second, F.fd_v)
-                              : fm::vel_update_sum(kv, v_m, vn_x, m_mm + m_m, a_mm + a_m, AL_mm + AL_m, div, cor, ext, imt, exb, imb, per_second);
+                second = upd_v(v_m, vn_x, TAKE ? 0.0 : m_mm + m_m, TAKE ? 0.0 : a_mm + a_m, AL_mm + AL_m, div, cor, ext, imt, exb, imb, per_second, F.fd_v);
             }
             first = W_0;
             XW_next = XW_0;
         } else {
             double W_0;
             {
-                const double ubar = fm::avg4(u_m, from_right(u_m), u_0, from_right(u_0));
+                const double ubar = fm::avg4(u_m, NBR ? uR_m : from_right(u_m), u_0, NBR ? uR_0 : from_right(u_0));
                 double div;
                 if constexpr (FULL) div = div2_full(false);
                 else div = fm::div2<UNI>(pc(T, FC_Q1N, r), vk(T, FC_Q2N, r, VK_Q2N), pc(T, FC_Q1S, r),
@@ -308,8 +350,7 @@
                 else cor = -vk(T, FC_FV, r, VK_FV) * ubar;
                 if (F.extra & 1) cor += F.xc_v;
                 if (F.extra & 2) div = fm::fma_(2.0, F.xd_v, div);
-                W_0 = F.fd ? fm::vel_update_sum_fd(kv, v_0, vn_x, m_m + m_0, a_m + a_0, AL_m + AL_0, div, cor, ext, imt, exb, imb, per_first, F.fd_v)
-                           : fm::vel_update_sum(kv, v_0, vn_x, m_m + m_0, a_m + a_0, AL_m + AL_0, div, cor, ext, imt, exb, imb, per_first);
+                W_0 = upd_v(v_0, vn_x, TAKE ? 0.0 : m_m + m_0, TAKE ? 0.0 : a_m + a_0, AL_m + AL_0, div, cor, ext, imt, exb, imb, per_first, F.fd_v);
             }
             const double XW_0 = fm::sum2(from_left(W_0), W_0);
             {
@@ -328,8 +369,7 @@
                 else cor = vk(T, FC_FU, j, VK_FU) * vbar;
                 if (F.extra & 1) cor += F.xc_u;
                 if (F.extra & 2) div = fm::fma_(2.0, F.xd_u, div);
-                second = F.fd ? fm::vel_update_sum_fd(kv, u_m, un_m, Xm_m, Xa_m, XAL_m, div, cor, ext, imt, exb, imb, per_second, F.fd_u)
-                              : fm::vel_update_sum(kv, u_m, un_m, Xm_m, Xa_m, XAL_m, div, cor, ext, imt, exb, imb, per_second);
+                second = upd_u(u_m, un_m, Xm_m, Xa_m, XAL_m, div, cor, ext, imt, exb, imb, per_second, F.fd_u);
             }
             first = W_0;
             XW_next = XW_0;
@@ -337,11 +377,15 @@
         SPROBE(sp3);
     }
 
+    template <bool TAKE = false>
     __device__ __forceinline__ void shift(double u_p, double v_p, double m_0, double a_0) {
         u_m = u_0; u_0 = u_p; v_m = v_0; v_0 = v_p;
+        if constexpr (NBR) { uR_m = uR_0; uR_0 = uR_p; }
         Xv_m = Xv_0; Xv_0 = Xv_p;
+        if constexpr (!TAKE) {
         a_mm = a_m; a_m = a_0; m_mm = m_m; m_m = m_0;
         Xm_m = Xm_0; Xa_m = Xa_0;
+        }
         e12_0 = e12_p;
         S11_mm = S11_m; S22_mm = S22_m; S12_mm = S12_m; AL_mm = AL_m;
         S11_m = S11_0; S22_m = S22_0; S12_m = S12_0; AL_m = AL_0;
```

Measured after the change: 69.90 billion cell-updates/s. 1.6% lower.
